# hermeznetwork/circuits

Measured on AMD Instinct MI355X. Metric: rollup-main tx-witnesses/sec (nTx=2048, nLevels=32), higher is better.
Workload: dtype u32x9 (254-bit Montgomery Fr, 29-bit limbs, integer)

## Files before the change

### circuits_amd/csrc/gen/poseidon_consts.inc

```

HZ_CONST_ARR uint32_t HZ_POSEIDON_K_T2[273][9] = {
  {0x01594cdfu, 0x0d359126u, 0x0974b8fau, 0x1c003576u, 0x02471552u, 0x01b4ec3eu, 0x0039cae5u, 0x0c4fdabeu, 0x001abb87u},
  {0x16429dadu, 0x10e8bfb1u, 0x0a355acau, 0x00ddcf00u, 0x157bd068u, 0x1f4bd7c1u, 0x10962bb4u, 0x16de36d0u, 0x000dca6eu},
  {0x1413967du, 0x105a9005u, 0x1046a4bcu, 0x1adfd419u, 0x03171c11u, 0x1a93314fu, 0x19defdc3u, 0x122f21d6u, 0x002ccaaau},
  {0x0c61afc0u, 0x056779b4u, 0x0dee0ab2u, 0x0375598cu, 0x1d6d65a3u, 0x1613901du, 0x0470c410u, 0x1b17f0fau, 0x0012ce74u},
  {0x17380b70u, 0x18b79fd8u, 0x0fff2f50u, 0x1ebcbaa5u, 0x1321aa93u, 0x0b639280u, 0x1f974844u, 0x1c31c015u, 0x00108ac7u},
  {0x1e193ea3u, 0x0edfdd9cu, 0x0997b975u, 0x0df6c0b5u, 0x0217b61fu, 0x19525ecfu, 0x1ab696fau, 0x1fc7b146u, 0x00284e43u},
  {0x1f60828fu, 0x05af232eu, 0x1e6e6a24u, 0x17b52dcau, 0x18396513u, 0x18a70df4u, 0x1ed87095u, 0x1edad4b1u, 0x002aea83u},
  {0x02cda9fbu, 0x1bf0915eu, 0x142bbe4du, 0x13dec3f2u, 0x15bd005fu, 0x1e47caf5u, 0x09d42d28u, 0x1c1453e2u, 0x00070815u},
  {0x0147b227u, 0x043db0d1u, 0x109123eeu, 0x02a96560u, 0x0545d476u, 0x16cafed6u, 0x06a7cde1u, 0x1b289bc1u, 0x000e717bu},
  {0x1245b46cu, 0x05baf901u, 0x158ae172u, 0x02c66a39u, 0x00422146u, 0x0330f8c1u, 0x18ebd100u, 0x083ed501u, 0x00045cd6u},
  {0x1fedd587u, 0x1762b199u, 0x188f8a60u, 0x1a6d7755u, 0x15ecf9b6u, 0x157d5954u, 0x0635d4eau, 0x15bef90du, 0x000f95b8u},
  {0x05977713u, 0x0322e34cu, 0x1952f2aau, 0x160cbb13u, 0x07d0a3afu, 0x0832dff0u, 0x032268dfu, 0x1dd156a4u, 0x00173356u},
  {0x1245b46cu, 0x05baf901u, 0x158ae172u, 0x02c66a39u, 0x00422146u, 0x0330f8c1u, 0x18ebd100u, 0x083ed501u, 0x00045cd6u},
  {0x0a443be3u, 0x0da43148u, 0x0d5bf075u, 0x0aec1b78u, 0x1aaeb7a0u, 0x1ecc745cu, 0x04cf1420u, 0x0dc2926au, 0x002568ccu},
  {0x091b4afcu, 0x1a830c13u, 0x07e0ffd2u, 0x13f0c21au, 0x032af443u, 0x059069deu, 0x00ee1d30u, 0x0b25f8dbu, 0x0023d9c4u},
  {0x199694a7u, 0x12ec6b8au, 0x1aa8f867u, 0x19c45019u, 0x16073cf7u, 0x14374c37u, 0x12acf9a0u, 0x14cc62ffu, 0x001c5cb3u},
  {0x18770d43u, 0x182a6057u, 0x1092ef6bu, 0x1b2c6b34u, 0x0d976099u, 0x09d7d0d6u, 0x10d8175cu, 0x0c978fadu, 0x001490ebu},
  {0x0193c086u, 0x1b408393u, 0x1f3f022au, 0x1a31c81bu, 0x189d54f9u, 0x068b8aa3u, 0x155b774fu, 0x1039e765u, 0x000ba3a7u},
  {0x1245b46cu, 0x05baf901u, 0x158ae172u, 0x02c66a39u, 0x00422146u, 0x0330f8c1u, 0x18ebd100u, 0x083ed501u, 0x00045cd6u},
  {0x1af15785u, 0x11f831e1u, 0x0267daa0u, 0x10300e25u, 0x03e3c029u, 0x0ba31833u, 0x1a77ab80u, 0x10a61ff1u, 0x002819c0u},
  {0x1c17b04du, 0x1e94304eu, 0x068d4e10u, 0x020b4caau, 0x1eae52eeu, 0x1709787au, 0x1d5718cdu, 0x06da8c2cu, 0x000510dfu},
  {0x1245b46cu, 0x05baf901u, 0x158ae172u, 0x02c66a39u, 0x00422146u, 0x0330f8c1u, 0x18ebd100u, 0x083ed501u, 0x00045cd6u},
  {0x034dc162u, 0x1240944bu, 0x11d0aab7u, 0x086e29ddu, 0x0bb57ea5u, 0x1be7bdc5u, 0x1830536bu, 0x0c707f25u, 0x001bae17u},
// ... 444 lines not shown
  {0x0ce9ef2fu, 0x1cccefd1u, 0x107971f9u, 0x18e2974du, 0x08e0fe13u, 0x11069f65u, 0x151cff07u, 0x0529a73cu, 0x0010af75u},
  {0x1c1a175fu, 0x0f3c9877u, 0x0e21d476u, 0x02ac34d1u, 0x0dfef3d2u, 0x064230f2u, 0x08129fddu, 0x18bd622fu, 0x000735e2u},
  {0x0dc8d1cbu, 0x036b8f33u, 0x01ed6b8cu, 0x1eb3968cu, 0x13a7f955u, 0x0864079au, 0x11167e93u, 0x13cb42b8u, 0x0020bc87u},
  {0x13c5e91bu, 0x0ba87ac2u, 0x1b35dd64u, 0x07cee755u, 0x1c0db2ccu, 0x10376d2cu, 0x1fc67e58u, 0x094ac052u, 0x000577e2u},
  {0x06bbddfcu, 0x14337540u, 0x1dc094e9u, 0x124bb7f4u, 0x0e6021a2u, 0x071160b8u, 0x18095154u, 0x02c8ef7fu, 0x002ed3cfu},
  {0x03f43b85u, 0x157841e5u, 0x10c98963u, 0x0418998bu, 0x1937d25eu, 0x0932adcdu, 0x0b54eefbu, 0x131462c1u, 0x0009c178u},
  {0x0ce9ef2fu, 0x1cccefd1u, 0x107971f9u, 0x18e2974du, 0x08e0fe13u, 0x11069f65u, 0x151cff07u, 0x0529a73cu, 0x0010af75u},
  {0x15ee3677u, 0x0c13b231u, 0x144efa88u, 0x0de5b1bfu, 0x1efac993u, 0x151746a9u, 0x14fd0730u, 0x1c09daa0u, 0x001f7c89u},
  {0x1690d1feu, 0x0d1ddecau, 0x1246e6f2u, 0x0b286eedu, 0x1928779cu, 0x1730207cu, 0x03d27a06u, 0x09fc86f6u, 0x003044e2u},
  {0x0ce9ef2fu, 0x1cccefd1u, 0x107971f9u, 0x18e2974du, 0x08e0fe13u, 0x11069f65u, 0x151cff07u, 0x0529a73cu, 0x0010af75u},
  {0x0087dbb8u, 0x0b7f49a5u, 0x17213affu, 0x0169024cu, 0x1efaa808u, 0x1332e2b1u, 0x1c0209aau, 0x03b65ef1u, 0x0029ec7du},
  {0x0dc8d1cbu, 0x036b8f33u, 0x01ed6b8cu, 0x1eb3968cu, 0x13a7f955u, 0x0864079au, 0x11167e93u, 0x13cb42b8u, 0x0020bc87u},
  {0x146627c7u, 0x0ec2014bu, 0x13e3a4fau, 0x10f1fbddu, 0x0c6927bfu, 0x0603e549u, 0x0fdede6bu, 0x04a0114du, 0x002aa135u},
  {0x11130434u, 0x1b3593dfu, 0x19c2e3f3u, 0x191de17eu, 0x174e43cbu, 0x1d73e4a2u, 0x1c6a1356u, 0x090ff16cu, 0x000f7aa8u},
  {0x08c96b43u, 0x15d0d426u, 0x0e9c36cau, 0x101a01f3u, 0x03d48d13u, 0x1b65ca68u, 0x06f3651eu, 0x0e606749u, 0x00014c14u},
  {0x0ce9ef2fu, 0x1cccefd1u, 0x107971f9u, 0x18e2974du, 0x08e0fe13u, 0x11069f65u, 0x151cff07u, 0x0529a73cu, 0x0010af75u},
  {0x1590348du, 0x0b1a1ff0u, 0x0256b576u, 0x0801f689u, 0x175d0092u, 0x06665c08u, 0x1485782bu, 0x0e73a331u, 0x002fe3ecu},
  {0x1b83c1f2u, 0x19d4c354u, 0x09225cd3u, 0x0ff73684u, 0x1a4c9a94u, 0x10d56a72u, 0x048ba310u, 0x1ab2e381u, 0x002c28e9u},
  {0x0ce9ef2fu, 0x1cccefd1u, 0x107971f9u, 0x18e2974du, 0x08e0fe13u, 0x11069f65u, 0x151cff07u, 0x0529a73cu, 0x0010af75u},
  {0x00133bfau, 0x0e899482u, 0x0eafa64du, 0x1ec347e5u, 0x0b3022a6u, 0x0f4f5da0u, 0x03e4545cu, 0x03909282u, 0x002f21f3u},
  {0x0dc8d1cbu, 0x036b8f33u, 0x01ed6b8cu, 0x1eb3968cu, 0x13a7f955u, 0x0864079au, 0x11167e93u, 0x13cb42b8u, 0x0020bc87u},
  {0x0779bf45u, 0x0dd361a6u, 0x114d0302u, 0x1d99ba2eu, 0x186d96c5u, 0x0e36dc9bu, 0x0dcf48feu, 0x1764b264u, 0x000fe0d8u},
  {0x155dba0eu, 0x171c731du, 0x0254bd0au, 0x0e38ebf8u, 0x1826d936u, 0x1a2e087au, 0x028f2facu, 0x1818d078u, 0x00283d8fu},
  {0x01846aafu, 0x03b9a57bu, 0x0f853ed1u, 0x156290a3u, 0x1557be9du, 0x1eeaf251u, 0x0f091d44u, 0x1aab9607u, 0x00089540u},
  {0x0ce9ef2fu, 0x1cccefd1u, 0x107971f9u, 0x18e2974du, 0x08e0fe13u, 0x11069f65u, 0x151cff07u, 0x0529a73cu, 0x0010af75u},
  {0x0aa1dbc3u, 0x14246c75u, 0x1e92c5feu, 0x19c7bb79u, 0x17e27b1du, 0x03f63d37u, 0x0a5d7805u, 0x029841f0u, 0x00082508u},
  {0x03149936u, 0x1f4f4b58u, 0x036104acu, 0x0d90df77u, 0x1716bfedu, 0x1fc8ce86u, 0x02f08225u, 0x074de8acu, 0x00268975u},
  {0x0ce9ef2fu, 0x1cccefd1u, 0x107971f9u, 0x18e2974du, 0x08e0fe13u, 0x11069f65u, 0x151cff07u, 0x0529a73cu, 0x0010af75u},
  {0x0f5596bdu, 0x07513a04u, 0x0be93490u, 0x105ceda5u, 0x09fe80edu, 0x0877ae07u, 0x0ec7a8c6u, 0x1c232985u, 0x002b00bfu},
  {0x0dc8d1cbu, 0x036b8f33u, 0x01ed6b8cu, 0x1eb3968cu, 0x13a7f955u, 0x0864079au, 0x11167e93u, 0x13cb42b8u, 0x0020bc87u},
  {0x16437a6fu, 0x12c5b47bu, 0x1c93eaabu, 0x0bbd1e23u, 0x0ee22d48u, 0x1a99f7ebu, 0x15913e64u, 0x1dbb478bu, 0x00138eadu},
  {0x1f7e1439u, 0x149868dcu, 0x1f3b7c70u, 0x085dd519u, 0x0df0faeau, 0x0c708ff4u, 0x1b3b42a3u, 0x0bb6177fu, 0x00203dcau},
  {0x020ef880u, 0x00aafe94u, 0x01b7bdeau, 0x044c0255u, 0x10f47161u, 0x0450224eu, 0x0a400180u, 0x0b851294u, 0x0018b435u},
  {0x0ce9ef2fu, 0x1cccefd1u, 0x107971f9u, 0x18e2974du, 0x08e0fe13u, 0x11069f65u, 0x151cff07u, 0x0529a73cu, 0x0010af75u},
  {0x0de9c761u, 0x06a21215u, 0x1860e3d0u, 0x1f62786au, 0x1e3ea970u, 0x1ebef040u, 0x0aa65466u, 0x0c3b5683u, 0x0003ee23u},
  {0x145fe787u, 0x00a69c58u, 0x06ffd046u, 0x0586dc35u, 0x0a74d8feu, 0x03266d07u, 0x1af54ed5u, 0x06086d0du, 0x0020c1aeu},
  {0x0ce9ef2fu, 0x1cccefd1u, 0x107971f9u, 0x18e2974du, 0x08e0fe13u, 0x11069f65u, 0x151cff07u, 0x0529a73cu, 0x0010af75u},
  {0x090f1c1au, 0x1dd1e152u, 0x081b956cu, 0x04e3453bu, 0x1ea8f4f6u, 0x02418e5eu, 0x07e022d7u, 0x13bf2ad6u, 0x002275dfu},
  {0x0dc8d1cbu, 0x036b8f33u, 0x01ed6b8cu, 0x1eb3968cu, 0x13a7f955u, 0x0864079au, 0x11167e93u, 0x13cb42b8u, 0x0020bc87u},
  {0x0c1abb13u, 0x1728bdfdu, 0x15074f4au, 0x1a70c65bu, 0x0372a452u, 0x13b51389u, 0x0c3abc69u, 0x0d4a70f3u, 0x0020073au},
  {0x0c2b5d5du, 0x0941df31u, 0x1f9c33bbu, 0x12962a4au, 0x0b917d15u, 0x185a5840u, 0x115784bfu, 0x09080cb2u, 0x000ed415u},
  {0x1775dec2u, 0x15289770u, 0x1c6088a0u, 0x0328b2cdu, 0x11c9218cu, 0x09ef8fc2u, 0x155805e3u, 0x130dcaf3u, 0x000f5a16u},
  {0x0ce9ef2fu, 0x1cccefd1u, 0x107971f9u, 0x18e2974du, 0x08e0fe13u, 0x11069f65u, 0x151cff07u, 0x0529a73cu, 0x0010af75u},
  {0x0f294db4u, 0x060e52fdu, 0x120959ebu, 0x157fdcaeu, 0x0155a8feu, 0x0ca01c37u, 0x03d8b2b0u, 0x0f6f8eeeu, 0x000bb5c3u},
  {0x19a3d3d4u, 0x05c86045u, 0x03d80b84u, 0x1363785cu, 0x0f8cace7u, 0x19750e68u, 0x1c95a3a0u, 0x0b0e3662u, 0x00176155u},
  {0x0ce9ef2fu, 0x1cccefd1u, 0x107971f9u, 0x18e2974du, 0x08e0fe13u, 0x11069f65u, 0x151cff07u, 0x0529a73cu, 0x0010af75u},
  {0x1cdf1c80u, 0x00af0c60u, 0x08f7f367u, 0x05d60c7fu, 0x17e5893cu, 0x0b71ee70u, 0x06987078u, 0x0a699221u, 0x000c359eu},
  {0x0dc8d1cbu, 0x036b8f33u, 0x01ed6b8cu, 0x1eb3968cu, 0x13a7f955u, 0x0864079au, 0x11167e93u, 0x13cb42b8u, 0x0020bc87u},
  {0x187f3b33u, 0x07888857u, 0x02795407u, 0x1f1a4efdu, 0x19cc12ceu, 0x1717fdbdu, 0x1ba7cd83u, 0x0be67905u, 0x00183a79u},
  {0x0a36210du, 0x0bb8a001u, 0x0309ec54u, 0x1a447634u, 0x0f7b6bd7u, 0x04421841u, 0x08805700u, 0x1d4e450bu, 0x00222d33u},
  {0x09ae6794u, 0x03440e85u, 0x03a40f4eu, 0x17aa9436u, 0x0e496c44u, 0x0f93daa8u, 0x0cc6d964u, 0x057a7f72u, 0x00260f79u},
  {0x0ce9ef2fu, 0x1cccefd1u, 0x107971f9u, 0x18e2974du, 0x08e0fe13u, 0x11069f65u, 0x151cff07u, 0x0529a73cu, 0x0010af75u},
  {0x0fe6dd74u, 0x188d3386u, 0x128b4934u, 0x011e4e6fu, 0x178eef24u, 0x01803342u, 0x12b47976u, 0x0ca4122bu, 0x001c86d1u},
  {0x029ab811u, 0x07e39ec6u, 0x1377f398u, 0x07111883u, 0x1565a2b6u, 0x05a895dcu, 0x0c719d0bu, 0x0b6ec86cu, 0x00299cd0u},
  {0x0ce9ef2fu, 0x1cccefd1u, 0x107971f9u, 0x18e2974du, 0x08e0fe13u, 0x11069f65u, 0x151cff07u, 0x0529a73cu, 0x0010af75u},
  {0x13b2c28au, 0x1d65d05au, 0x0669f2a2u, 0x1c2cf4c7u, 0x0558d099u, 0x006d7b4bu, 0x0fd78bb9u, 0x1c3432ceu, 0x002e725cu},
  {0x0dc8d1cbu, 0x036b8f33u, 0x01ed6b8cu, 0x1eb3968cu, 0x13a7f955u, 0x0864079au, 0x11167e93u, 0x13cb42b8u, 0x0020bc87u},
  {0x002ace2bu, 0x082d7fd9u, 0x100eb90bu, 0x05fd2ab3u, 0x0a2ab5a7u, 0x0c503845u, 0x104b1988u, 0x0d86a39eu, 0x00134db8u},
  {0x07e6e8d9u, 0x1f13b995u, 0x1cae0afcu, 0x098a0d09u, 0x12962c84u, 0x0aa5d7a0u, 0x0378ce02u, 0x177cbab4u, 0x000bf75au},
  {0x1e90d55fu, 0x0c21c683u, 0x0a8fdb6eu, 0x026d43d3u, 0x0e390d06u, 0x0d6c90e7u, 0x168d4726u, 0x095549d8u, 0x002a185du},
  {0x0ce9ef2fu, 0x1cccefd1u, 0x107971f9u, 0x18e2974du, 0x08e0fe13u, 0x11069f65u, 0x151cff07u, 0x0529a73cu, 0x0010af75u},
  {0x1fbddbf4u, 0x1304aa18u, 0x088f5eedu, 0x19402e89u, 0x1297e6cdu, 0x1a825ea2u, 0x0f19dcf8u, 0x07a72d6eu, 0x002c1983u},
  {0x07f633bfu, 0x1f9c2a8bu, 0x13a4ce2eu, 0x02ab1954u, 0x0b4efa3au, 0x16ed044fu, 0x0146aa31u, 0x18a3ba03u, 0x0022d34eu},
  {0x0ce9ef2fu, 0x1cccefd1u, 0x107971f9u, 0x18e2974du, 0x08e0fe13u, 0x11069f65u, 0x151cff07u, 0x0529a73cu, 0x0010af75u},
  {0x019b67d0u, 0x164636dcu, 0x126a234au, 0x16d1b300u, 0x1c910526u, 0x0ce66e11u, 0x1e3651e9u, 0x065d025fu, 0x001c3089u},
  {0x0dc8d1cbu, 0x036b8f33u, 0x01ed6b8cu, 0x1eb3968cu, 0x13a7f955u, 0x0864079au, 0x11167e93u, 0x13cb42b8u, 0x0020bc87u},
  {0x0cad4af9u, 0x0b68dc9au, 0x0521d195u, 0x0ca35a05u, 0x1f992f30u, 0x085c9779u, 0x0d2de48bu, 0x1978f12au, 0x0008c9e0u},
  {0x09800555u, 0x113d463bu, 0x069e7f85u, 0x12a0ff18u, 0x14f170a4u, 0x1d0dcc14u, 0x08d21537u, 0x1443adf8u, 0x00293740u},
  {0x00209e79u, 0x0f3754d1u, 0x0a372977u, 0x0af44dacu, 0x1556b961u, 0x02079085u, 0x1689cb71u, 0x062b1b95u, 0x00282c23u},
  {0x1ebad59bu, 0x0303e4d1u, 0x1f9a501eu, 0x0371d097u, 0x1121228bu, 0x030ff9cbu, 0x1669aeebu, 0x17074050u, 0x00167af6u},
  {0x08dedc9cu, 0x105fdd77u, 0x0e4cdd32u, 0x169a2ae2u, 0x183b48d1u, 0x13008989u, 0x1120efb6u, 0x00964973u, 0x001a5077u},
  {0x0db2b350u, 0x12e399dau, 0x0a131677u, 0x029e66cau, 0x05c4c5dfu, 0x0cf59ec0u, 0x15fa74f4u, 0x0fa03f09u, 0x001d5589u},
  {0x08e6a481u, 0x1c20cbc0u, 0x1c586468u, 0x1773f1dfu, 0x1ea21907u, 0x1d0ad80eu, 0x1c95d935u, 0x154be0d5u, 0x000ba91fu},
  {0x1ac99e79u, 0x0b5f4be9u, 0x1916cf2au, 0x0f819302u, 0x023ab1cau, 0x041f93b2u, 0x09cdbbe5u, 0x1fc8875bu, 0x001cd993u},
  {0x0e58f564u, 0x1eef6bf8u, 0x1944e2b1u, 0x164add07u, 0x1b83d866u, 0x17f8882au, 0x1aee24c8u, 0x0691d0ccu, 0x000b299bu},
  {0x1d695ae1u, 0x1c431d9au, 0x1c1f930eu, 0x033e4eb3u, 0x198cfc7bu, 0x1e26027cu, 0x066653dcu, 0x047b3c5bu, 0x000e649eu},
  {0x1f96ed35u, 0x0f49c18fu, 0x1dbb6db8u, 0x1b10e15au, 0x0449aa7du, 0x1e72fce1u, 0x036b8328u, 0x1eb8c773u, 0x0023f542u},
  {0x0ce9ef2fu, 0x1cccefd1u, 0x107971f9u, 0x18e2974du, 0x08e0fe13u, 0x11069f65u, 0x151cff07u, 0x0529a73cu, 0x0010af75u},
  {0x0d9ab9d7u, 0x0ca84190u, 0x04829da9u, 0x132817e3u, 0x17a45765u, 0x1ea14297u, 0x00eb3e80u, 0x061685f7u, 0x001016feu},
  {0x1a861e2du, 0x0e651276u, 0x0ef852f4u, 0x10c58332u, 0x0c3674f3u, 0x16090e81u, 0x0d596687u, 0x1f438e1cu, 0x0013949cu},
  {0x06f7520fu, 0x09d4f250u, 0x15681fe9u, 0x01fcd044u, 0x105154f2u, 0x1a33cff0u, 0x14edfb9fu, 0x19bb1130u, 0x0008a998u},
};
#define HZ_POSEIDON_RP_T2 56
HZ_CONST_ARR uint32_t HZ_POSEIDON_K_T3[407][9] = {
  {0x06950af2u, 0x08df52acu, 0x1f463fb0u, 0x0afd92f8u, 0x14c68fb5u, 0x085357afu, 0x17f37f7du, 0x1a172af8u, 0x00219b98u},
  {0x14ac6331u, 0x19c5c962u, 0x14d4d232u, 0x1b75b979u, 0x05cb57afu, 0x1631c351u, 0x1539ab4eu, 0x0ae57f69u, 0x00221b93u},
  {0x0a11b110u, 0x0dfeef5cu, 0x0072b018u, 0x1dd64482u, 0x001637a2u, 0x1ccbb6f7u, 0x1bfe61e2u, 0x125c529fu, 0x0001ce06u},
  {0x00249cd2u, 0x182cbeffu, 0x156efbbdu, 0x0eba1325u, 0x06ee80ddu, 0x1457c2ebu, 0x0be3d716u, 0x1eff46fcu, 0x00136e88u},
  {0x1072044du, 0x05806d3bu, 0x069a7439u, 0x1dc94561u, 0x0aefed59u, 0x00905741u, 0x049e47f4u, 0x09217d14u, 0x0009b22fu},
  {0x0422baecu, 0x1338c9abu, 0x10cb4a50u, 0x0f33676cu, 0x10e8f39au, 0x12776997u, 0x0d5d7ea2u, 0x1b2dc6aau, 0x002038dfu},
  {0x17bad917u, 0x06dec5c8u, 0x0e531d76u, 0x0c62440bu, 0x147b04a7u, 0x1355af66u, 0x15363704u, 0x06bbd64au, 0x0029f279u},
  {0x0746570du, 0x01d97fc5u, 0x155c6647u, 0x0d79b529u, 0x1b39ce8cu, 0x14086985u, 0x1a8401efu, 0x05c9ac6du, 0x000199b3u},
  {0x09ebbb6cu, 0x1881a596u, 0x181e6e0fu, 0x1fabcdc3u, 0x088b122eu, 0x114f31d0u, 0x0fb3243eu, 0x09ac2ff3u, 0x0012841au},
  {0x1cfff79eu, 0x03d7755du, 0x0552bbd3u, 0x12213286u, 0x09228c55u, 0x0bef4aebu, 0x13fe8d05u, 0x17692838u, 0x00036614u},
  {0x11317367u, 0x1d4e5366u, 0x09855a5du, 0x0c1df16du, 0x0b0de371u, 0x0d9605ccu, 0x0adb0fa5u, 0x1329da0bu, 0x00227fdeu},
  {0x08acea5fu, 0x0838fb1bu, 0x1a12541au, 0x0a38ec24u, 0x02af6162u, 0x188f221fu, 0x19735f0fu, 0x04e9316eu, 0x000e33f9u},
  {0x071e41a6u, 0x08bbea5fu, 0x065da30bu, 0x0228a38au, 0x076a9fb7u, 0x1a1469bdu, 0x114c885eu, 0x110fd199u, 0x001b4b49u},
  {0x0f9e7ad7u, 0x110388bbu, 0x0b23a8beu, 0x0d3738ecu, 0x067c9996u, 0x106d3f50u, 0x0b10e901u, 0x0ec1ca43u, 0x00185422u},
  {0x1d808d1bu, 0x1da4b2b8u, 0x1a384bf5u, 0x0f4905bau, 0x03e20d93u, 0x0012de4fu, 0x121bce86u, 0x16d26544u, 0x000ade3au},
  {0x132d35feu, 0x16391cd7u, 0x16fa00a5u, 0x0bb956dbu, 0x1caed5d5u, 0x1b6e4830u, 0x0a6f14e8u, 0x07466b6cu, 0x00191d6cu},
  {0x012e70d0u, 0x0da73962u, 0x1ec66759u, 0x09107002u, 0x033f84eeu, 0x1399f16eu, 0x0226a56eu, 0x08d116b4u, 0x000e6296u},
  {0x0f9e7ad7u, 0x110388bbu, 0x0b23a8beu, 0x0d3738ecu, 0x067c9996u, 0x106d3f50u, 0x0b10e901u, 0x0ec1ca43u, 0x00185422u},
  {0x0bb951acu, 0x06443faau, 0x17ed611cu, 0x1884421cu, 0x1afce51fu, 0x0efea9e7u, 0x147f1ed0u, 0x0c2df3cfu, 0x00136fbcu},
  {0x1fe33105u, 0x0c4a3c3cu, 0x1c2cdf0fu, 0x041c6828u, 0x048b6c4au, 0x0719d197u, 0x123ecde6u, 0x05abf637u, 0x002ba99eu},
  {0x1137c2e7u, 0x189c540cu, 0x02a348f5u, 0x178dc616u, 0x16997355u, 0x01b921a7u, 0x0fa7ff5fu, 0x02545751u, 0x0009f1ecu},
  {0x13599399u, 0x141ae82bu, 0x13ee16cbu, 0x1358b994u, 0x1601460au, 0x144e8e2fu, 0x0bfd8788u, 0x17aa03a2u, 0x002ae961u},
  {0x05212230u, 0x1c5e5216u, 0x117426b0u, 0x0de4f9e8u, 0x0851a05au, 0x18c6202bu, 0x09247701u, 0x110886d9u, 0x002cb167u},
  {0x18349cb5u, 0x0e276a55u, 0x0cde03c9u, 0x0a96a06cu, 0x02315530u, 0x02cc974fu, 0x15fc8764u, 0x05814578u, 0x0014a31cu},
  {0x03effa5du, 0x162ae321u, 0x14e1d723u, 0x0c68e230u, 0x16cd0944u, 0x1bbee942u, 0x0c6310ddu, 0x11183e90u, 0x002c6b1au},
  {0x05e1c028u, 0x07e01aecu, 0x066688e6u, 0x025ed81cu, 0x14304feau, 0x058a629du, 0x0d6605aeu, 0x173ec4edu, 0x00105204u},
  {0x0f9e7ad7u, 0x110388bbu, 0x0b23a8beu, 0x0d3738ecu, 0x067c9996u, 0x106d3f50u, 0x0b10e901u, 0x0ec1ca43u, 0x00185422u},
  {0x1181abafu, 0x1777b75eu, 0x028f3017u, 0x1c94d28fu, 0x10777d08u, 0x05a1b685u, 0x0a46f0f9u, 0x1e0f866cu, 0x001dbad8u},
  {0x0b3ea51cu, 0x03c81aebu, 0x067c2073u, 0x08738320u, 0x0d32836du, 0x01e483dbu, 0x11cc9a33u, 0x069d55c4u, 0x000f80f1u},
  {0x0fc51587u, 0x0e287af7u, 0x13e1b330u, 0x111abc40u, 0x129058d3u, 0x06ef59b7u, 0x1ea08cafu, 0x0b61be00u, 0x001ec76au},
  {0x0f9e7ad7u, 0x110388bbu, 0x0b23a8beu, 0x0d3738ecu, 0x067c9996u, 0x106d3f50u, 0x0b10e901u, 0x0ec1ca43u, 0x00185422u},
  {0x0df0fb39u, 0x1aa3a276u, 0x1b2456bcu, 0x0b0b4edeu, 0x1ba9e05au, 0x15f65f18u, 0x15794d20u, 0x0cc2d3ecu, 0x00076bd6u},
  {0x13142375u, 0x14870790u, 0x00255288u, 0x1c96ff90u, 0x1fa42dccu, 0x0052b5aau, 0x0670de46u, 0x0cbb0d43u, 0x00260ef0u},
  {0x1137c2e7u, 0x189c540cu, 0x02a348f5u, 0x178dc616u, 0x16997355u, 0x01b921a7u, 0x0fa7ff5fu, 0x02545751u, 0x0009f1ecu},
  {0x0c3aa2dbu, 0x036876d2u, 0x05cbc67bu, 0x162a139du, 0x028bba81u, 0x1b0b894eu, 0x1d398215u, 0x1843792bu, 0x0025435fu},
  {0x08a19517u, 0x1781c4e2u, 0x17c032b7u, 0x0cf6014cu, 0x125fbbc2u, 0x00be09e1u, 0x0291a374u, 0x1080ee7bu, 0x000d2661u},
  {0x044def6eu, 0x15147e38u, 0x060ea740u, 0x0e96aac6u, 0x00fce055u, 0x1356abd6u, 0x1d59ef48u, 0x04b5c547u, 0x00025392u},
  {0x13c28a85u, 0x1744f037u, 0x199f241bu, 0x195989b8u, 0x07693e3bu, 0x09727d90u, 0x000ec272u, 0x0031339au, 0x0011656eu},
  {0x004f4c98u, 0x12aeff7bu, 0x14a4ee7au, 0x189c6531u, 0x1807b4d1u, 0x1fb90164u, 0x0fe8359eu, 0x05aa0bdeu, 0x00143e04u},
  {0x0f9e7ad7u, 0x110388bbu, 0x0b23a8beu, 0x0d3738ecu, 0x067c9996u, 0x106d3f50u, 0x0b10e901u, 0x0ec1ca43u, 0x00185422u},
  {0x0a741350u, 0x1f77effbu, 0x1cdce38au, 0x0658a913u, 0x03783795u, 0x0937fefau, 0x08eeb4f3u, 0x005c1b6au, 0x001188feu},
  {0x09b423d8u, 0x031ea254u, 0x042feb00u, 0x1da37bd7u, 0x140c6fc8u, 0x14a61766u, 0x1745a732u, 0x11d84ceeu, 0x0028ae3fu},
  {0x10751df5u, 0x19b4cf5cu, 0x0bc089e2u, 0x19248dbau, 0x160c19b3u, 0x14de6553u, 0x12ee493cu, 0x097bb0e2u, 0x001dc890u},
  {0x0f9e7ad7u, 0x110388bbu, 0x0b23a8beu, 0x0d3738ecu, 0x067c9996u, 0x106d3f50u, 0x0b10e901u, 0x0ec1ca43u, 0x00185422u},
  {0x193adc08u, 0x16078c77u, 0x06d56e91u, 0x03c2a1efu, 0x1c365a79u, 0x0fd772eau, 0x0827e9eeu, 0x190172bbu, 0x002fd5b0u},
  {0x124638d1u, 0x19c9ba46u, 0x0d3b1c7cu, 0x137e8f4du, 0x03d39810u, 0x1aea945eu, 0x18beb131u, 0x054c38f6u, 0x002e492cu},
  {0x1137c2e7u, 0x189c540cu, 0x02a348f5u, 0x178dc616u, 0x16997355u, 0x01b921a7u, 0x0fa7ff5fu, 0x02545751u, 0x0009f1ecu},
  {0x0ed76c01u, 0x1f2b360au, 0x09540f46u, 0x16ea79a2u, 0x1eb62a52u, 0x0ee0687au, 0x1c4b333bu, 0x1155e835u, 0x001fa7c7u},
  {0x00372895u, 0x04170c43u, 0x1b4cdaa3u, 0x100289ffu, 0x0ed8eb5bu, 0x04452cc9u, 0x02813767u, 0x10470445u, 0x00272319u},
  {0x1c1e81cfu, 0x0e6f1ad7u, 0x1e80f9d4u, 0x0dc77746u, 0x16c3884bu, 0x04e75b8du, 0x07ae2c07u, 0x194253a0u, 0x0004e551u},
  {0x015e9592u, 0x0b0b67c9u, 0x0a6040d5u, 0x1e2118c3u, 0x142bc4ddu, 0x0b213b29u, 0x0ec11bddu, 0x1c2440c0u, 0x000b5732u},
  {0x00b22627u, 0x126f6426u, 0x1ffdba02u, 0x0f2a6ba7u, 0x09a16dfau, 0x1a4f249bu, 0x10de2db9u, 0x0be04320u, 0x00142a4cu},
  {0x0f9e7ad7u, 0x110388bbu, 0x0b23a8beu, 0x0d3738ecu, 0x067c9996u, 0x106d3f50u, 0x0b10e901u, 0x0ec1ca43u, 0x00185422u},
  {0x07d56552u, 0x14c10409u, 0x1bff85c4u, 0x13994671u, 0x0218ce8cu, 0x1070f8dbu, 0x185823d5u, 0x100e7753u, 0x0000847fu},
  {0x16c11742u, 0x14ee17d2u, 0x18e7742eu, 0x0e7c9b5eu, 0x129b3fd1u, 0x020bb1aeu, 0x05569922u, 0x0f07b878u, 0x0017ad0eu},
  {0x03b9a38eu, 0x187e8f4fu, 0x0d3cc940u, 0x03b09c80u, 0x15f75dd3u, 0x160d0e6au, 0x1de9da2bu, 0x115a1843u, 0x00053acbu},
  {0x0f9e7ad7u, 0x110388bbu, 0x0b23a8beu, 0x0d3738ecu, 0x067c9996u, 0x106d3f50u, 0x0b10e901u, 0x0ec1ca43u, 0x00185422u},
  {0x0a0e5b99u, 0x112c0bdau, 0x136ec440u, 0x011bda31u, 0x1e8293b3u, 0x0ed8fffeu, 0x16228411u, 0x1eb9c0a8u, 0x000408f7u},
  {0x0136b0e6u, 0x1b782ae9u, 0x0d4b2341u, 0x09c51220u, 0x0fb1b417u, 0x0135e40eu, 0x08349207u, 0x04817981u, 0x000424ebu},
  {0x1137c2e7u, 0x189c540cu, 0x02a348f5u, 0x178dc616u, 0x16997355u, 0x01b921a7u, 0x0fa7ff5fu, 0x02545751u, 0x0009f1ecu},
  {0x1c058a5cu, 0x11f0f414u, 0x1881b744u, 0x1ea573eeu, 0x0568c0c0u, 0x1461d0f2u, 0x16c672acu, 0x04bf6096u, 0x00115f9au},
  {0x0b3d2dbbu, 0x1f73b37eu, 0x1bdaa8bbu, 0x1dffb532u, 0x1b62d93cu, 0x05493558u, 0x0f951a50u, 0x0f84ad81u, 0x00081e33u},
  {0x19f6b4ddu, 0x1878eef4u, 0x126a20b0u, 0x16fc2d48u, 0x0a7e56cbu, 0x0e4ef340u, 0x0d473220u, 0x0c9d56eeu, 0x0025a632u},
  {0x1bfe70f2u, 0x02b15e7du, 0x0ce8c95du, 0x0a8521ecu, 0x02f9df40u, 0x1cc38b7eu, 0x1d945fb6u, 0x060c100eu, 0x0018f902u},
  {0x18270344u, 0x0b57920fu, 0x1b9c93fdu, 0x03ac7f4cu, 0x1947743bu, 0x17506abbu, 0x16afd566u, 0x1c7dd946u, 0x001fed53u},
  {0x0f9e7ad7u, 0x110388bbu, 0x0b23a8beu, 0x0d3738ecu, 0x067c9996u, 0x106d3f50u, 0x0b10e901u, 0x0ec1ca43u, 0x00185422u},
  {0x1fe0a28du, 0x00078f50u, 0x1478d6e3u, 0x1c0326afu, 0x0134abc1u, 0x14749a6du, 0x1fccfb03u, 0x074f7280u, 0x001afe92u},
  {0x1ddb71d8u, 0x0d176c28u, 0x1a7b6a60u, 0x0e11e3ecu, 0x194df12bu, 0x05fa7958u, 0x0a9400b7u, 0x0dcf9cc5u, 0x0008b5c6u},
  {0x0285585bu, 0x0f4a048du, 0x04237b8fu, 0x1ea6a0e8u, 0x161e90f3u, 0x1e60de4fu, 0x1c3a0eaau, 0x165f0cbeu, 0x00296fc6u},
  {0x0f9e7ad7u, 0x110388bbu, 0x0b23a8beu, 0x0d3738ecu, 0x067c9996u, 0x106d3f50u, 0x0b10e901u, 0x0ec1ca43u, 0x00185422u},
  {0x148bfc35u, 0x0cf89969u, 0x16538c96u, 0x1908b913u, 0x0c80f272u, 0x05cc9d74u, 0x02d2f02eu, 0x1d2c6174u, 0x00269fddu},
  {0x082101f0u, 0x093d5a3cu, 0x1ac61b3du, 0x0ada0389u, 0x02515da2u, 0x0b400f9bu, 0x0879a4a3u, 0x0bfc5fd0u, 0x0011bb73u},
  {0x1137c2e7u, 0x189c540cu, 0x02a348f5u, 0x178dc616u, 0x16997355u, 0x01b921a7u, 0x0fa7ff5fu, 0x02545751u, 0x0009f1ecu},
  {0x1d3c64bcu, 0x03073507u, 0x02a12d0fu, 0x0003f27cu, 0x1f24e51du, 0x1254b14fu, 0x0bee568fu, 0x16003172u, 0x000c42c1u},
  {0x1bddc0d0u, 0x01fd0077u, 0x1bb32ba3u, 0x0715d62cu, 0x05e80565u, 0x15ab3c30u, 0x133f8882u, 0x01185f69u, 0x0017ea3cu},
  {0x0d003002u, 0x0c6e38c7u, 0x0339d8e1u, 0x063769d3u, 0x0b5b9b6eu, 0x1628a5acu, 0x1bbc7ee2u, 0x172584d5u, 0x0001a051u},
  {0x12d02f2bu, 0x1152fc47u, 0x04cb874du, 0x17491130u, 0x1d2e57f2u, 0x0e523b31u, 0x1b098b80u, 0x047d4272u, 0x00267465u},
  {0x1c195f82u, 0x00ce598du, 0x1d0f727fu, 0x07588154u, 0x141ee2dcu, 0x14894b4du, 0x1c441381u, 0x1dd39709u, 0x001bef96u},
  {0x0f9e7ad7u, 0x110388bbu, 0x0b23a8beu, 0x0d3738ecu, 0x067c9996u, 0x106d3f50u, 0x0b10e901u, 0x0ec1ca43u, 0x00185422u},
  {0x1a1739ceu, 0x0f45c151u, 0x02f6c2a2u, 0x0784afa0u, 0x1e3392e7u, 0x04e8f2bdu, 0x091ec827u, 0x10918acdu, 0x002c0081u},
  {0x19836dbfu, 0x1b96e774u, 0x14a9d05fu, 0x1d13244bu, 0x0a5d02c8u, 0x19a2dc16u, 0x092eea4bu, 0x137c7dcbu, 0x000d4079u},
  {0x040174f4u, 0x1c9bcfa0u, 0x1d68236au, 0x1449d35cu, 0x03856edbu, 0x1b6df7a1u, 0x0a6de30cu, 0x089526beu, 0x00183d2fu},
  {0x0f9e7ad7u, 0x110388bbu, 0x0b23a8beu, 0x0d3738ecu, 0x067c9996u, 0x106d3f50u, 0x0b10e901u, 0x0ec1ca43u, 0x00185422u},
// ... 241 lines not shown
  {0x04504510u, 0x0f45d601u, 0x01ecc1b2u, 0x05390587u, 0x18fe614cu, 0x03b9c159u, 0x0e1699b9u, 0x17312ca8u, 0x002c6582u},
  {0x0f9e7ad7u, 0x110388bbu, 0x0b23a8beu, 0x0d3738ecu, 0x067c9996u, 0x106d3f50u, 0x0b10e901u, 0x0ec1ca43u, 0x00185422u},
  {0x17decd6cu, 0x1b512009u, 0x1e9f9256u, 0x19771112u, 0x01f3a959u, 0x02f1eca2u, 0x16707e6fu, 0x111a7d2au, 0x001c8454u},
  {0x1d64b848u, 0x0387544cu, 0x19aa56fdu, 0x0eb4d623u, 0x11edaae2u, 0x16ad2ff1u, 0x07b2692au, 0x167fe61bu, 0x001c6befu},
  {0x1107f769u, 0x13e86f43u, 0x0e096f08u, 0x1d15b2ebu, 0x0583b869u, 0x13dd21dbu, 0x1304cce1u, 0x0a7853a8u, 0x0022f768u},
  {0x0f9e7ad7u, 0x110388bbu, 0x0b23a8beu, 0x0d3738ecu, 0x067c9996u, 0x106d3f50u, 0x0b10e901u, 0x0ec1ca43u, 0x00185422u},
  {0x0d78d317u, 0x0b44e42du, 0x05b02ac4u, 0x15aba253u, 0x1add0fc7u, 0x10327e73u, 0x1ea22c2au, 0x080e44a1u, 0x001db63au},
  {0x054a0314u, 0x087b0914u, 0x16253cf8u, 0x1c9ad78bu, 0x01ed4c61u, 0x0c3a2206u, 0x05de0913u, 0x035ad09fu, 0x002bd824u},
  {0x1137c2e7u, 0x189c540cu, 0x02a348f5u, 0x178dc616u, 0x16997355u, 0x01b921a7u, 0x0fa7ff5fu, 0x02545751u, 0x0009f1ecu},
  {0x16ce8bdbu, 0x0982e0e6u, 0x0f90c5beu, 0x1003a2d6u, 0x1603772au, 0x17d87051u, 0x0f760d39u, 0x015064dbu, 0x001ea2afu},
  {0x106eee6bu, 0x1b1ba868u, 0x169c9c24u, 0x1ff77aa4u, 0x1f68f059u, 0x088f515du, 0x15db4f59u, 0x020b4215u, 0x001541a8u},
  {0x0b2bb3a0u, 0x11f35cf2u, 0x152ff881u, 0x0106230du, 0x0b6d3097u, 0x12149d4du, 0x1116ab6eu, 0x04e4853fu, 0x00085941u},
  {0x0a327e91u, 0x114ba57cu, 0x17d82f7cu, 0x0ef9b1d0u, 0x0134d8fcu, 0x018601e1u, 0x0fff4bb4u, 0x10d507cbu, 0x000f398eu},
  {0x17d2a5f8u, 0x1be95064u, 0x14c2725fu, 0x1cd1e4d0u, 0x01cbaef2u, 0x16ead87du, 0x03e536f9u, 0x0ae8b949u, 0x000c406au},
  {0x0f9e7ad7u, 0x110388bbu, 0x0b23a8beu, 0x0d3738ecu, 0x067c9996u, 0x106d3f50u, 0x0b10e901u, 0x0ec1ca43u, 0x00185422u},
  {0x0c8c189cu, 0x1cc79ae9u, 0x186f6aecu, 0x105d0b36u, 0x01f9589eu, 0x111a0c4eu, 0x09f087f6u, 0x1f316c99u, 0x001e9076u},
  {0x0c8e3650u, 0x0a732d7cu, 0x10ce5b06u, 0x16b2ab83u, 0x19f98e8fu, 0x0c94e3f7u, 0x05f604ceu, 0x1a8b8e0du, 0x0021178du},
  {0x1401e080u, 0x1beb9ea3u, 0x02266b39u, 0x174e8dbcu, 0x1730b2dfu, 0x00f38faau, 0x042c2d23u, 0x1d877771u, 0x0017c9c6u},
  {0x0f9e7ad7u, 0x110388bbu, 0x0b23a8beu, 0x0d3738ecu, 0x067c9996u, 0x106d3f50u, 0x0b10e901u, 0x0ec1ca43u, 0x00185422u},
  {0x1f884e54u, 0x0b9c236fu, 0x0ffa2cfau, 0x0e54ca2du, 0x010c2515u, 0x19c42314u, 0x09e3bc58u, 0x0be5373au, 0x00112560u},
  {0x0ec7d1f5u, 0x087eae30u, 0x1e043f6du, 0x1be1c3a3u, 0x08da1a2du, 0x09b47136u, 0x0e53ffb3u, 0x0a866559u, 0x0016d8a7u},
  {0x1137c2e7u, 0x189c540cu, 0x02a348f5u, 0x178dc616u, 0x16997355u, 0x01b921a7u, 0x0fa7ff5fu, 0x02545751u, 0x0009f1ecu},
  {0x1da30c2cu, 0x0f5d2c4cu, 0x11a6cde7u, 0x116b4311u, 0x1809871au, 0x137d501cu, 0x1123dc35u, 0x1391dbf6u, 0x002d1005u},
  {0x0db8d418u, 0x1adb76f8u, 0x127c029au, 0x14b7d9bdu, 0x17ad4c8bu, 0x17ca7b0du, 0x1d702f41u, 0x1fa8eba5u, 0x002bf205u},
  {0x071418f5u, 0x03adff73u, 0x17631518u, 0x10e4a5efu, 0x0a7296eeu, 0x17fca3f3u, 0x178a4dfdu, 0x0da5e8cau, 0x00012346u},
  {0x11e77690u, 0x13e71dd7u, 0x01d14895u, 0x1db5672du, 0x11b62312u, 0x1cbca505u, 0x093ab4d0u, 0x18eee72eu, 0x001d24f6u},
  {0x09ee2a2du, 0x0ee1c318u, 0x1128c87au, 0x116c5524u, 0x0d79df55u, 0x01c1c1fau, 0x0057112du, 0x1b2fc7d5u, 0x0008fad4u},
  {0x0f9e7ad7u, 0x110388bbu, 0x0b23a8beu, 0x0d3738ecu, 0x067c9996u, 0x106d3f50u, 0x0b10e901u, 0x0ec1ca43u, 0x00185422u},
  {0x01b412a1u, 0x11517daau, 0x00540991u, 0x0113f263u, 0x0cad8dc0u, 0x1e38c735u, 0x1083c0b1u, 0x0454a866u, 0x002de93du},
  {0x066867cbu, 0x1709d8f6u, 0x1268dab4u, 0x1ebf2c12u, 0x04525e2au, 0x15291888u, 0x0572ee91u, 0x169b6e4au, 0x00037f15u},
  {0x0c52838du, 0x1f7616ddu, 0x1ff2c2b6u, 0x0e5b5312u, 0x04fd5bc5u, 0x140fd5f5u, 0x0931bc69u, 0x07ecf7ffu, 0x0010e5b8u},
  {0x0f9e7ad7u, 0x110388bbu, 0x0b23a8beu, 0x0d3738ecu, 0x067c9996u, 0x106d3f50u, 0x0b10e901u, 0x0ec1ca43u, 0x00185422u},
  {0x104007c0u, 0x1973ae9au, 0x17e72900u, 0x1375271bu, 0x1a446a16u, 0x1c953efbu, 0x07d7a070u, 0x1aa59967u, 0x0017f2e5u},
  {0x10581566u, 0x0f7c6f29u, 0x04914c1fu, 0x097c1a30u, 0x11540718u, 0x1b3acacbu, 0x1972e53du, 0x0ce1cb37u, 0x0030293fu},
  {0x1137c2e7u, 0x189c540cu, 0x02a348f5u, 0x178dc616u, 0x16997355u, 0x01b921a7u, 0x0fa7ff5fu, 0x02545751u, 0x0009f1ecu},
  {0x188e3de4u, 0x1f555a7eu, 0x1dd46cdeu, 0x1c6c3570u, 0x1eed9cf2u, 0x0dc8763au, 0x1004454eu, 0x0de3e924u, 0x002f4e33u},
  {0x0c5f88d3u, 0x03e3096au, 0x0f277f99u, 0x002d9412u, 0x0380edcdu, 0x1cf049eau, 0x07298468u, 0x15b6041eu, 0x0009a103u},
  {0x1ea662b3u, 0x19e9c268u, 0x0b673a2fu, 0x0ee34c9cu, 0x0bda421bu, 0x1da6c94du, 0x027e3ec2u, 0x17cf8091u, 0x0011895cu},
  {0x033c4532u, 0x11a0da34u, 0x0e6adaecu, 0x0cf2a6f9u, 0x0ba128b9u, 0x006f2f72u, 0x08cb767du, 0x0b83f781u, 0x000550ecu},
  {0x08083788u, 0x132bf382u, 0x06ab3f3fu, 0x0f45e3c8u, 0x0dd4e47fu, 0x11eeea60u, 0x0704743eu, 0x0d6b3a26u, 0x0009ea97u},
  {0x0f9e7ad7u, 0x110388bbu, 0x0b23a8beu, 0x0d3738ecu, 0x067c9996u, 0x106d3f50u, 0x0b10e901u, 0x0ec1ca43u, 0x00185422u},
  {0x01a5bfb3u, 0x0d5d2e82u, 0x0585a98fu, 0x1607f9f1u, 0x16813062u, 0x0a23f347u, 0x0813c376u, 0x0802503bu, 0x0008fdc2u},
  {0x00645c3cu, 0x05f5f813u, 0x1665816au, 0x1c33f6afu, 0x0fee29c9u, 0x18321ba5u, 0x1a7f3602u, 0x1226e7aeu, 0x0010c633u},
  {0x077a7aafu, 0x174787c6u, 0x16e776d5u, 0x09061190u, 0x17368f18u, 0x0dde5cbeu, 0x10269ba5u, 0x1cc9a02fu, 0x000286f5u},
  {0x0f9e7ad7u, 0x110388bbu, 0x0b23a8beu, 0x0d3738ecu, 0x067c9996u, 0x106d3f50u, 0x0b10e901u, 0x0ec1ca43u, 0x00185422u},
  {0x05e28124u, 0x1b9981d7u, 0x16ae361cu, 0x04bc466bu, 0x1e9aa74bu, 0x1777bd70u, 0x1eb5a877u, 0x1b915a64u, 0x00263302u},
  {0x04736068u, 0x1e6524e9u, 0x0234ea3eu, 0x094ffe5du, 0x12bb81f9u, 0x1c13536eu, 0x02b9f33au, 0x1c536667u, 0x000f5a14u},
  {0x1137c2e7u, 0x189c540cu, 0x02a348f5u, 0x178dc616u, 0x16997355u, 0x01b921a7u, 0x0fa7ff5fu, 0x02545751u, 0x0009f1ecu},
  {0x0a854573u, 0x1ece4e1bu, 0x1a96a584u, 0x1f741153u, 0x17ecba0du, 0x16b912c0u, 0x1f3f28abu, 0x13878f8bu, 0x001478e0u},
  {0x10aaa709u, 0x128030d5u, 0x09db228cu, 0x19a4911fu, 0x10214415u, 0x1d699a6du, 0x1f89f93fu, 0x1ab05164u, 0x00115707u},
  {0x19612a18u, 0x0624738cu, 0x0304ed35u, 0x1a932dccu, 0x039b436bu, 0x093ed15fu, 0x0f91e976u, 0x10efa55fu, 0x000c1d91u},
  {0x1d4373ffu, 0x0885b851u, 0x13bc85ffu, 0x07a97785u, 0x0e01a209u, 0x0a882789u, 0x14f27303u, 0x1f6a17a0u, 0x001f687eu},
  {0x14f3dba6u, 0x1c57a0f3u, 0x15231329u, 0x0906d34cu, 0x1276e7a4u, 0x0647ccb0u, 0x079deceau, 0x1954f267u, 0x001673a3u},
  {0x0f9e7ad7u, 0x110388bbu, 0x0b23a8beu, 0x0d3738ecu, 0x067c9996u, 0x106d3f50u, 0x0b10e901u, 0x0ec1ca43u, 0x00185422u},
  {0x0d1778f7u, 0x041b88deu, 0x08ed1482u, 0x1ab09f93u, 0x11db568fu, 0x1f90934eu, 0x0bd90f32u, 0x07ae718bu, 0x0014be32u},
  {0x18767531u, 0x123587e3u, 0x16cf2177u, 0x0b7a27d5u, 0x199c91e6u, 0x18344467u, 0x1f23001au, 0x1b67428cu, 0x00165fedu},
  {0x04035ab7u, 0x009c7862u, 0x08f75c89u, 0x0e3fd310u, 0x0ddc22c1u, 0x0a209e57u, 0x07e87572u, 0x1a8c9221u, 0x00119157u},
  {0x128dc94bu, 0x19758516u, 0x0b627578u, 0x05c780e8u, 0x05319927u, 0x00faab0au, 0x1a439ee2u, 0x01f5011au, 0x002601a6u},
  {0x1b2e1d77u, 0x08ae3e44u, 0x1d2038d8u, 0x1e635985u, 0x1ae5d306u, 0x13d871bbu, 0x1fbdc1ddu, 0x0f2f62e6u, 0x000059b0u},
  {0x07e732fcu, 0x084df909u, 0x14efe205u, 0x15aa326du, 0x0a20fff7u, 0x17653bacu, 0x02a6c29bu, 0x0b2c5a75u, 0x001f3bc3u},
  {0x048acd07u, 0x03082733u, 0x1e26560au, 0x034af7a5u, 0x0bb2c60bu, 0x163a0e84u, 0x18607102u, 0x001dae37u, 0x002df20fu},
  {0x1600f2beu, 0x019cbdc4u, 0x05a53411u, 0x1d6cdfecu, 0x1739894fu, 0x12a7d77bu, 0x1c6b1d54u, 0x16a08d44u, 0x000bf852u},
  {0x0f99ded2u, 0x0e06bc02u, 0x06df134eu, 0x1578d322u, 0x149724d4u, 0x18c3bf95u, 0x00eae83au, 0x0c011e07u, 0x001750c4u},
  {0x02a052cau, 0x05a87ab0u, 0x14dcddbcu, 0x106decafu, 0x122e2ce8u, 0x03d4082eu, 0x0ef8f873u, 0x1521e336u, 0x0016a065u},
  {0x0df025bau, 0x0ba73f8eu, 0x0f915324u, 0x065bbda3u, 0x0ca80a7cu, 0x118624f1u, 0x09498173u, 0x01c7a1a4u, 0x000af019u},
  {0x05a499dcu, 0x12206bd0u, 0x0b814efbu, 0x0d66bfceu, 0x0e7dbb5cu, 0x0aa0171du, 0x08e70184u, 0x059ef913u, 0x001323dfu},
  {0x0649905eu, 0x17c95f8fu, 0x05a65489u, 0x13644fe0u, 0x0536260au, 0x0ace1d58u, 0x17055235u, 0x06869bfau, 0x001a7e62u},
  {0x0b45af89u, 0x0224c0c3u, 0x1bfb0ddbu, 0x0f9b48f9u, 0x17da019cu, 0x14f45fd8u, 0x10997d57u, 0x0f86e29eu, 0x0026efadu},
  {0x04565569u, 0x07905e05u, 0x1df8e797u, 0x06d4b35bu, 0x04ad02a2u, 0x0778a22fu, 0x01d1297eu, 0x1d84f2a0u, 0x0027fe28u},
  {0x0d82889au, 0x0fa45e0eu, 0x1bd530f5u, 0x1a53f924u, 0x05eb0d8au, 0x1b365b8bu, 0x1381f308u, 0x196c0c25u, 0x001bede7u},
  {0x0bec1d0cu, 0x04b3688eu, 0x18cf405fu, 0x0f800727u, 0x056de992u, 0x00fb9fd2u, 0x05514427u, 0x1fb2f130u, 0x0020c03fu},
  {0x01768fb6u, 0x18f63897u, 0x070ed03cu, 0x1a001f72u, 0x04ce0399u, 0x01841053u, 0x0b9737e5u, 0x09292366u, 0x0010faecu},
  {0x0751cdcau, 0x0fe2d7e2u, 0x0162e9f3u, 0x0b12636cu, 0x05f02906u, 0x1a592918u, 0x17c0c8beu, 0x003c4496u, 0x001a52bdu},
  {0x0e8efa33u, 0x0f51cc96u, 0x0edc3d40u, 0x12573aefu, 0x16b95ae8u, 0x1b7bf14fu, 0x011482afu, 0x16b1e719u, 0x00135a61u},
  {0x0f9e7ad7u, 0x110388bbu, 0x0b23a8beu, 0x0d3738ecu, 0x067c9996u, 0x106d3f50u, 0x0b10e901u, 0x0ec1ca43u, 0x00185422u},
  {0x1d808d1bu, 0x1da4b2b8u, 0x1a384bf5u, 0x0f4905bau, 0x03e20d93u, 0x0012de4fu, 0x121bce86u, 0x16d26544u, 0x000ade3au},
  {0x132d35feu, 0x16391cd7u, 0x16fa00a5u, 0x0bb956dbu, 0x1caed5d5u, 0x1b6e4830u, 0x0a6f14e8u, 0x07466b6cu, 0x00191d6cu},
  {0x18e9ba8fu, 0x1d8162aeu, 0x0fbf09d7u, 0x168662d1u, 0x0ef7b2feu, 0x015d7d55u, 0x09195718u, 0x0267a28cu, 0x000fe908u},
  {0x04f388d7u, 0x01b14590u, 0x1598e8a8u, 0x12c58329u, 0x115458c8u, 0x13a62935u, 0x03d65e2eu, 0x13e8407cu, 0x000ab495u},
  {0x0564e591u, 0x01d4df72u, 0x0b0ad8d6u, 0x1655ae03u, 0x13a1b5e6u, 0x0a93bc0du, 0x16ec5d74u, 0x1374ea59u, 0x002369d6u},
  {0x0004eaddu, 0x05365bf4u, 0x0493016eu, 0x1d1a2414u, 0x0c60826du, 0x023b2076u, 0x026fd3e9u, 0x055a47d6u, 0x0021dc8bu},
  {0x17fddfa0u, 0x161a5176u, 0x030d78bau, 0x15ef8400u, 0x08d839abu, 0x1b2dce76u, 0x14b8a677u, 0x07c85cffu, 0x000877ecu},
  {0x0e5224f4u, 0x1e27ada2u, 0x1eb9ae97u, 0x0a2f7a59u, 0x1f07c890u, 0x1a2da267u, 0x05d3f5a1u, 0x11654cdeu, 0x000ba411u},
};
HZ_CONST_ARR uint32_t HZ_POSEIDON_KW_T3[407][9] = {
  {0x06950af2u, 0x08df52acu, 0x1f463fb0u, 0x0afd92f8u, 0x14c68fb5u, 0x085357afu, 0x17f37f7du, 0x1a172af8u, 0x00219b98u},
  {0x14ac6331u, 0x19c5c962u, 0x14d4d232u, 0x1b75b979u, 0x05cb57afu, 0x1631c351u, 0x1539ab4eu, 0x0ae57f69u, 0x00221b93u},
  {0x0a11b110u, 0x0dfeef5cu, 0x0072b018u, 0x1dd64482u, 0x001637a2u, 0x1ccbb6f7u, 0x1bfe61e2u, 0x125c529fu, 0x0001ce06u},
  {0x00249cd2u, 0x182cbeffu, 0x156efbbdu, 0x0eba1325u, 0x06ee80ddu, 0x1457c2ebu, 0x0be3d716u, 0x1eff46fcu, 0x00136e88u},
  {0x1072044du, 0x05806d3bu, 0x069a7439u, 0x1dc94561u, 0x0aefed59u, 0x00905741u, 0x049e47f4u, 0x09217d14u, 0x0009b22fu},
  {0x0422baecu, 0x1338c9abu, 0x10cb4a50u, 0x0f33676cu, 0x10e8f39au, 0x12776997u, 0x0d5d7ea2u, 0x1b2dc6aau, 0x002038dfu},
  {0x17bad917u, 0x06dec5c8u, 0x0e531d76u, 0x0c62440bu, 0x147b04a7u, 0x1355af66u, 0x15363704u, 0x06bbd64au, 0x0029f279u},
  {0x0746570du, 0x01d97fc5u, 0x155c6647u, 0x0d79b529u, 0x1b39ce8cu, 0x14086985u, 0x1a8401efu, 0x05c9ac6du, 0x000199b3u},
  {0x09ebbb6cu, 0x1881a596u, 0x181e6e0fu, 0x1fabcdc3u, 0x088b122eu, 0x114f31d0u, 0x0fb3243eu, 0x09ac2ff3u, 0x0012841au},
  {0x1cfff79eu, 0x03d7755du, 0x0552bbd3u, 0x12213286u, 0x09228c55u, 0x0bef4aebu, 0x13fe8d05u, 0x17692838u, 0x00036614u},
  {0x11317367u, 0x1d4e5366u, 0x09855a5du, 0x0c1df16du, 0x0b0de371u, 0x0d9605ccu, 0x0adb0fa5u, 0x1329da0bu, 0x00227fdeu},
  {0x08acea5fu, 0x0838fb1bu, 0x1a12541au, 0x0a38ec24u, 0x02af6162u, 0x188f221fu, 0x19735f0fu, 0x04e9316eu, 0x000e33f9u},
  {0x071e41a6u, 0x08bbea5fu, 0x065da30bu, 0x0228a38au, 0x076a9fb7u, 0x1a1469bdu, 0x114c885eu, 0x110fd199u, 0x001b4b49u},
  {0x1a4711d7u, 0x16699559u, 0x1c235d50u, 0x0b4e4a8eu, 0x14df94adu, 0x0965c795u, 0x1d7afd37u, 0x0342cc8du, 0x002d76dbu},
  {0x1d808d1bu, 0x1da4b2b8u, 0x1a384bf5u, 0x0f4905bau, 0x03e20d93u, 0x0012de4fu, 0x121bce86u, 0x16d26544u, 0x000ade3au},
  {0x132d35feu, 0x16391cd7u, 0x16fa00a5u, 0x0bb956dbu, 0x1caed5d5u, 0x1b6e4830u, 0x0a6f14e8u, 0x07466b6cu, 0x00191d6cu},
  {0x012e70d0u, 0x0da73962u, 0x1ec66759u, 0x09107002u, 0x033f84eeu, 0x1399f16eu, 0x0226a56eu, 0x08d116b4u, 0x000e6296u},
  {0x1a4711d7u, 0x16699559u, 0x1c235d50u, 0x0b4e4a8eu, 0x14df94adu, 0x0965c795u, 0x1d7afd37u, 0x0342cc8du, 0x002d76dbu},
  {0x0bb951acu, 0x06443faau, 0x17ed611cu, 0x1884421cu, 0x1afce51fu, 0x0efea9e7u, 0x147f1ed0u, 0x0c2df3cfu, 0x00136fbcu},
  {0x1fe33105u, 0x0c4a3c3cu, 0x1c2cdf0fu, 0x041c6828u, 0x048b6c4au, 0x0719d197u, 0x123ecde6u, 0x05abf637u, 0x002ba99eu},
  {0x068a4cfdu, 0x1fd63110u, 0x13da84bdu, 0x0a050f73u, 0x028bc9fcu, 0x1f7d6d37u, 0x06270e37u, 0x18ff0e31u, 0x001cf5b4u},
  {0x13599399u, 0x141ae82bu, 0x13ee16cbu, 0x1358b994u, 0x1601460au, 0x144e8e2fu, 0x0bfd8788u, 0x17aa03a2u, 0x002ae961u},
  {0x14725df5u, 0x1b005648u, 0x0162c706u, 0x0531cd6du, 0x02a601f6u, 0x165a1032u, 0x162de27fu, 0x05fe8aa5u, 0x002ddc1bu},
  {0x1726ad0au, 0x1fd8b292u, 0x09a1fb0fu, 0x151b5e74u, 0x0fe81d33u, 0x06afb3b4u, 0x0d979567u, 0x02e791a9u, 0x000c050bu},
  {0x196992a9u, 0x1d5a94c8u, 0x1c410c4cu, 0x1872c758u, 0x06ccf87au, 0x050d05b8u, 0x0620aa0eu, 0x1febdc6au, 0x000503fdu},
  {0x14832d19u, 0x0c864124u, 0x142a6f13u, 0x1d21efa1u, 0x12b9569eu, 0x066ca828u, 0x044dcb54u, 0x02a472afu, 0x002ee064u},
  {0x1a4711d7u, 0x16699559u, 0x1c235d50u, 0x0b4e4a8eu, 0x14df94adu, 0x0965c795u, 0x1d7afd37u, 0x0342cc8du, 0x002d76dbu},
  {0x1181abafu, 0x1777b75eu, 0x028f3017u, 0x1c94d28fu, 0x10777d08u, 0x05a1b685u, 0x0a46f0f9u, 0x1e0f866cu, 0x001dbad8u},
  {0x0b3ea51cu, 0x03c81aebu, 0x067c2073u, 0x08738320u, 0x0d32836du, 0x01e483dbu, 0x11cc9a33u, 0x069d55c4u, 0x000f80f1u},
  {0x0fc51587u, 0x0e287af7u, 0x13e1b330u, 0x111abc40u, 0x129058d3u, 0x06ef59b7u, 0x1ea08cafu, 0x0b61be00u, 0x001ec76au},
  {0x1a4711d7u, 0x16699559u, 0x1c235d50u, 0x0b4e4a8eu, 0x14df94adu, 0x0965c795u, 0x1d7afd37u, 0x0342cc8du, 0x002d76dbu},
  {0x0df0fb39u, 0x1aa3a276u, 0x1b2456bcu, 0x0b0b4edeu, 0x1ba9e05au, 0x15f65f18u, 0x15794d20u, 0x0cc2d3ecu, 0x00076bd6u},
  {0x13142375u, 0x14870790u, 0x00255288u, 0x1c96ff90u, 0x1fa42dccu, 0x0052b5aau, 0x0670de46u, 0x0cbb0d43u, 0x00260ef0u},
  {0x068a4cfdu, 0x1fd63110u, 0x13da84bdu, 0x0a050f73u, 0x028bc9fcu, 0x1f7d6d37u, 0x06270e37u, 0x18ff0e31u, 0x001cf5b4u},
  {0x0c3aa2dbu, 0x036876d2u, 0x05cbc67bu, 0x162a139du, 0x028bba81u, 0x1b0b894eu, 0x1d398215u, 0x1843792bu, 0x0025435fu},
  {0x137a33b7u, 0x03f5fbbbu, 0x121af88eu, 0x1d01a9f8u, 0x0d6390b5u, 0x026b6983u, 0x0413bb1bu, 0x1856e380u, 0x000d084fu},
  {0x1d0d9ecbu, 0x097a305fu, 0x01130901u, 0x10506c2bu, 0x0896c878u, 0x16684f5au, 0x1aa3ac6bu, 0x119611f1u, 0x00118237u},
  {0x12d676c8u, 0x06ed38b8u, 0x017fa970u, 0x0ed10765u, 0x1f0efb44u, 0x0a05ba6cu, 0x03e3151bu, 0x14e1bd7au, 0x001dc77bu},
  {0x18219b9bu, 0x1954cd82u, 0x13d500cau, 0x182aa853u, 0x0a6d8b14u, 0x0cde9933u, 0x17244744u, 0x19c86591u, 0x002459b7u},
  {0x1a4711d7u, 0x16699559u, 0x1c235d50u, 0x0b4e4a8eu, 0x14df94adu, 0x0965c795u, 0x1d7afd37u, 0x0342cc8du, 0x002d76dbu},
  {0x0a741350u, 0x1f77effbu, 0x1cdce38au, 0x0658a913u, 0x03783795u, 0x0937fefau, 0x08eeb4f3u, 0x005c1b6au, 0x001188feu},
  {0x09b423d8u, 0x031ea254u, 0x042feb00u, 0x1da37bd7u, 0x140c6fc8u, 0x14a61766u, 0x1745a732u, 0x11d84ceeu, 0x0028ae3fu},
  {0x10751df5u, 0x19b4cf5cu, 0x0bc089e2u, 0x19248dbau, 0x160c19b3u, 0x14de6553u, 0x12ee493cu, 0x097bb0e2u, 0x001dc890u},
  {0x1a4711d7u, 0x16699559u, 0x1c235d50u, 0x0b4e4a8eu, 0x14df94adu, 0x0965c795u, 0x1d7afd37u, 0x0342cc8du, 0x002d76dbu},
  {0x193adc08u, 0x16078c77u, 0x06d56e91u, 0x03c2a1efu, 0x1c365a79u, 0x0fd772eau, 0x0827e9eeu, 0x190172bbu, 0x002fd5b0u},
  {0x124638d1u, 0x19c9ba46u, 0x0d3b1c7cu, 0x137e8f4du, 0x03d39810u, 0x1aea945eu, 0x18beb131u, 0x054c38f6u, 0x002e492cu},
  {0x068a4cfdu, 0x1fd63110u, 0x13da84bdu, 0x0a050f73u, 0x028bc9fcu, 0x1f7d6d37u, 0x06270e37u, 0x18ff0e31u, 0x001cf5b4u},
  {0x0ed76c01u, 0x1f2b360au, 0x09540f46u, 0x16ea79a2u, 0x1eb62a52u, 0x0ee0687au, 0x1c4b333bu, 0x1155e835u, 0x001fa7c7u},
  {0x0c84cfb7u, 0x0f60856fu, 0x01250caau, 0x03df44b0u, 0x0a88cc23u, 0x089a9e40u, 0x199df927u, 0x197e3d72u, 0x00090b50u},
  {0x07ed5296u, 0x08309766u, 0x13d285ddu, 0x101efe56u, 0x18535a20u, 0x04b4e7a8u, 0x18e7fa88u, 0x15feb658u, 0x0021dae6u},
  {0x0f4ab17fu, 0x1133e7ceu, 0x0eb88ffbu, 0x15087e81u, 0x1a7eadadu, 0x1d0a26b1u, 0x1957d717u, 0x0d7bcd9fu, 0x001f589eu},
  {0x06462a0du, 0x02b7344bu, 0x0ad5c140u, 0x1af91cb0u, 0x0ddd502fu, 0x0a37b18cu, 0x045c4737u, 0x1c40f96eu, 0x0011c7c8u},
  {0x1a4711d7u, 0x16699559u, 0x1c235d50u, 0x0b4e4a8eu, 0x14df94adu, 0x0965c795u, 0x1d7afd37u, 0x0342cc8du, 0x002d76dbu},
  {0x07d56552u, 0x14c10409u, 0x1bff85c4u, 0x13994671u, 0x0218ce8cu, 0x1070f8dbu, 0x185823d5u, 0x100e7753u, 0x0000847fu},
  {0x16c11742u, 0x14ee17d2u, 0x18e7742eu, 0x0e7c9b5eu, 0x129b3fd1u, 0x020bb1aeu, 0x05569922u, 0x0f07b878u, 0x0017ad0eu},
  {0x03b9a38eu, 0x187e8f4fu, 0x0d3cc940u, 0x03b09c80u, 0x15f75dd3u, 0x160d0e6au, 0x1de9da2bu, 0x115a1843u, 0x00053acbu},
  {0x1a4711d7u, 0x16699559u, 0x1c235d50u, 0x0b4e4a8eu, 0x14df94adu, 0x0965c795u, 0x1d7afd37u, 0x0342cc8du, 0x002d76dbu},
  {0x0a0e5b99u, 0x112c0bdau, 0x136ec440u, 0x011bda31u, 0x1e8293b3u, 0x0ed8fffeu, 0x16228411u, 0x1eb9c0a8u, 0x000408f7u},
  {0x0136b0e6u, 0x1b782ae9u, 0x0d4b2341u, 0x09c51220u, 0x0fb1b417u, 0x0135e40eu, 0x08349207u, 0x04817981u, 0x000424ebu},
  {0x068a4cfdu, 0x1fd63110u, 0x13da84bdu, 0x0a050f73u, 0x028bc9fcu, 0x1f7d6d37u, 0x06270e37u, 0x18ff0e31u, 0x001cf5b4u},
  {0x1c058a5cu, 0x11f0f414u, 0x1881b744u, 0x1ea573eeu, 0x0568c0c0u, 0x1461d0f2u, 0x16c672acu, 0x04bf6096u, 0x00115f9au},
  {0x094ebfd4u, 0x0d47c9a8u, 0x15ea20f3u, 0x08317642u, 0x170adfcau, 0x1fcd5fcbu, 0x04c99096u, 0x111c32aau, 0x002e5c83u},
  {0x1802183eu, 0x07e52223u, 0x1446cd28u, 0x15e69cbfu, 0x02ced7a1u, 0x0de9a90eu, 0x0535631eu, 0x0f20adffu, 0x000d259bu},
  {0x1d308172u, 0x0ad59071u, 0x085cb467u, 0x1e36a0bdu, 0x04198146u, 0x1a21c1c8u, 0x0b64b510u, 0x0b0adc5du, 0x0025dd52u},
  {0x1e2da772u, 0x00835255u, 0x0955e640u, 0x09c71077u, 0x1a87db02u, 0x04d66f25u, 0x1ec156d8u, 0x12625712u, 0x001dcc16u},
  {0x1a4711d7u, 0x16699559u, 0x1c235d50u, 0x0b4e4a8eu, 0x14df94adu, 0x0965c795u, 0x1d7afd37u, 0x0342cc8du, 0x002d76dbu},
  {0x1fe0a28du, 0x00078f50u, 0x1478d6e3u, 0x1c0326afu, 0x0134abc1u, 0x14749a6du, 0x1fccfb03u, 0x074f7280u, 0x001afe92u},
  {0x1ddb71d8u, 0x0d176c28u, 0x1a7b6a60u, 0x0e11e3ecu, 0x194df12bu, 0x05fa7958u, 0x0a9400b7u, 0x0dcf9cc5u, 0x0008b5c6u},
  {0x0285585bu, 0x0f4a048du, 0x04237b8fu, 0x1ea6a0e8u, 0x161e90f3u, 0x1e60de4fu, 0x1c3a0eaau, 0x165f0cbeu, 0x00296fc6u},
  {0x1a4711d7u, 0x16699559u, 0x1c235d50u, 0x0b4e4a8eu, 0x14df94adu, 0x0965c795u, 0x1d7afd37u, 0x0342cc8du, 0x002d76dbu},
  {0x148bfc35u, 0x0cf89969u, 0x16538c96u, 0x1908b913u, 0x0c80f272u, 0x05cc9d74u, 0x02d2f02eu, 0x1d2c6174u, 0x00269fddu},
  {0x082101f0u, 0x093d5a3cu, 0x1ac61b3du, 0x0ada0389u, 0x02515da2u, 0x0b400f9bu, 0x0879a4a3u, 0x0bfc5fd0u, 0x0011bb73u},
  {0x068a4cfdu, 0x1fd63110u, 0x13da84bdu, 0x0a050f73u, 0x028bc9fcu, 0x1f7d6d37u, 0x06270e37u, 0x18ff0e31u, 0x001cf5b4u},
  {0x1d3c64bcu, 0x03073507u, 0x02a12d0fu, 0x0003f27cu, 0x1f24e51du, 0x1254b14fu, 0x0bee568fu, 0x16003172u, 0x000c42c1u},
  {0x0e28a5dfu, 0x14aaf111u, 0x01500700u, 0x17ae740bu, 0x1823e1abu, 0x0941469eu, 0x1cd9e9a3u, 0x089fcaa3u, 0x001a9340u},
  {0x1fe953dbu, 0x1b0550b2u, 0x113081e2u, 0x1ce1ad77u, 0x1cc23c0bu, 0x19862292u, 0x07da7441u, 0x14604074u, 0x00122b00u},
  {0x189360ccu, 0x00f4d6cfu, 0x05c64a62u, 0x041f5b88u, 0x09e749a9u, 0x06b022ddu, 0x0fba7039u, 0x083eca6cu, 0x002ad2b4u},
  {0x104fc2a8u, 0x1119d1c0u, 0x148ffc7eu, 0x127830eeu, 0x043bc94cu, 0x189532b9u, 0x0183862eu, 0x04ac30c8u, 0x000bf3fdu},
  {0x1a4711d7u, 0x16699559u, 0x1c235d50u, 0x0b4e4a8eu, 0x14df94adu, 0x0965c795u, 0x1d7afd37u, 0x0342cc8du, 0x002d76dbu},
  {0x1a1739ceu, 0x0f45c151u, 0x02f6c2a2u, 0x0784afa0u, 0x1e3392e7u, 0x04e8f2bdu, 0x091ec827u, 0x10918acdu, 0x002c0081u},
  {0x19836dbfu, 0x1b96e774u, 0x14a9d05fu, 0x1d13244bu, 0x0a5d02c8u, 0x19a2dc16u, 0x092eea4bu, 0x137c7dcbu, 0x000d4079u},
  {0x040174f4u, 0x1c9bcfa0u, 0x1d68236au, 0x1449d35cu, 0x03856edbu, 0x1b6df7a1u, 0x0a6de30cu, 0x089526beu, 0x00183d2fu},
  {0x1a4711d7u, 0x16699559u, 0x1c235d50u, 0x0b4e4a8eu, 0x14df94adu, 0x0965c795u, 0x1d7afd37u, 0x0342cc8du, 0x002d76dbu},
// ... 241 lines not shown
  {0x185c06e6u, 0x1acd2060u, 0x09f13546u, 0x1632c012u, 0x0adb560bu, 0x1f8f83fdu, 0x043970c4u, 0x090568b9u, 0x002bafe9u},
  {0x1a4711d7u, 0x16699559u, 0x1c235d50u, 0x0b4e4a8eu, 0x14df94adu, 0x0965c795u, 0x1d7afd37u, 0x0342cc8du, 0x002d76dbu},
  {0x17decd6cu, 0x1b512009u, 0x1e9f9256u, 0x19771112u, 0x01f3a959u, 0x02f1eca2u, 0x16707e6fu, 0x111a7d2au, 0x001c8454u},
  {0x1d64b848u, 0x0387544cu, 0x19aa56fdu, 0x0eb4d623u, 0x11edaae2u, 0x16ad2ff1u, 0x07b2692au, 0x167fe61bu, 0x001c6befu},
  {0x1107f769u, 0x13e86f43u, 0x0e096f08u, 0x1d15b2ebu, 0x0583b869u, 0x13dd21dbu, 0x1304cce1u, 0x0a7853a8u, 0x0022f768u},
  {0x1a4711d7u, 0x16699559u, 0x1c235d50u, 0x0b4e4a8eu, 0x14df94adu, 0x0965c795u, 0x1d7afd37u, 0x0342cc8du, 0x002d76dbu},
  {0x0d78d317u, 0x0b44e42du, 0x05b02ac4u, 0x15aba253u, 0x1add0fc7u, 0x10327e73u, 0x1ea22c2au, 0x080e44a1u, 0x001db63au},
  {0x054a0314u, 0x087b0914u, 0x16253cf8u, 0x1c9ad78bu, 0x01ed4c61u, 0x0c3a2206u, 0x05de0913u, 0x035ad09fu, 0x002bd824u},
  {0x068a4cfdu, 0x1fd63110u, 0x13da84bdu, 0x0a050f73u, 0x028bc9fcu, 0x1f7d6d37u, 0x06270e37u, 0x18ff0e31u, 0x001cf5b4u},
  {0x16ce8bdbu, 0x0982e0e6u, 0x0f90c5beu, 0x1003a2d6u, 0x1603772au, 0x17d87051u, 0x0f760d39u, 0x015064dbu, 0x001ea2afu},
  {0x1a011c44u, 0x0749d3adu, 0x19e7538fu, 0x127ace8bu, 0x075228a1u, 0x167999beu, 0x1d281b9bu, 0x009c7303u, 0x00109532u},
  {0x1a5cb872u, 0x1611fcf1u, 0x18eba770u, 0x135f5e04u, 0x07248222u, 0x04b684fcu, 0x188fc050u, 0x12d1f064u, 0x0018b335u},
  {0x0dfc7eeeu, 0x000279f5u, 0x1df140deu, 0x05fdd766u, 0x1dae1aeau, 0x0854346eu, 0x0c97665cu, 0x19c5a768u, 0x000eeb44u},
  {0x08694e5eu, 0x1da9de00u, 0x09edcd95u, 0x19d3b050u, 0x18b26442u, 0x09453651u, 0x1e4d9868u, 0x1853c5dfu, 0x001e2384u},
  {0x1a4711d7u, 0x16699559u, 0x1c235d50u, 0x0b4e4a8eu, 0x14df94adu, 0x0965c795u, 0x1d7afd37u, 0x0342cc8du, 0x002d76dbu},
  {0x0c8c189cu, 0x1cc79ae9u, 0x186f6aecu, 0x105d0b36u, 0x01f9589eu, 0x111a0c4eu, 0x09f087f6u, 0x1f316c99u, 0x001e9076u},
  {0x0c8e3650u, 0x0a732d7cu, 0x10ce5b06u, 0x16b2ab83u, 0x19f98e8fu, 0x0c94e3f7u, 0x05f604ceu, 0x1a8b8e0du, 0x0021178du},
  {0x1401e080u, 0x1beb9ea3u, 0x02266b39u, 0x174e8dbcu, 0x1730b2dfu, 0x00f38faau, 0x042c2d23u, 0x1d877771u, 0x0017c9c6u},
  {0x1a4711d7u, 0x16699559u, 0x1c235d50u, 0x0b4e4a8eu, 0x14df94adu, 0x0965c795u, 0x1d7afd37u, 0x0342cc8du, 0x002d76dbu},
  {0x1f884e54u, 0x0b9c236fu, 0x0ffa2cfau, 0x0e54ca2du, 0x010c2515u, 0x19c42314u, 0x09e3bc58u, 0x0be5373au, 0x00112560u},
  {0x0ec7d1f5u, 0x087eae30u, 0x1e043f6du, 0x1be1c3a3u, 0x08da1a2du, 0x09b47136u, 0x0e53ffb3u, 0x0a866559u, 0x0016d8a7u},
  {0x068a4cfdu, 0x1fd63110u, 0x13da84bdu, 0x0a050f73u, 0x028bc9fcu, 0x1f7d6d37u, 0x06270e37u, 0x18ff0e31u, 0x001cf5b4u},
  {0x1da30c2cu, 0x0f5d2c4cu, 0x11a6cde7u, 0x116b4311u, 0x1809871au, 0x137d501cu, 0x1123dc35u, 0x1391dbf6u, 0x002d1005u},
  {0x1bd0e9e8u, 0x16c855dbu, 0x122e30e2u, 0x0a45d15eu, 0x164b0017u, 0x00c91fb5u, 0x0b383caeu, 0x0192821du, 0x0027a242u},
  {0x061088e5u, 0x06ad42d3u, 0x1c3f9509u, 0x1e26bbd2u, 0x1d4b96f4u, 0x0029432cu, 0x0ac30fe0u, 0x106015e7u, 0x00012ff4u},
  {0x13387124u, 0x07da2b39u, 0x11632bccu, 0x1fa87b21u, 0x16cbe30au, 0x1c3a66e8u, 0x056b0585u, 0x1d20ee10u, 0x0013c2cau},
  {0x1c110a8du, 0x105aa29eu, 0x06b50424u, 0x01576549u, 0x046d2ba7u, 0x03f1043cu, 0x0e483368u, 0x0a83e681u, 0x001ccdbbu},
  {0x1a4711d7u, 0x16699559u, 0x1c235d50u, 0x0b4e4a8eu, 0x14df94adu, 0x0965c795u, 0x1d7afd37u, 0x0342cc8du, 0x002d76dbu},
  {0x01b412a1u, 0x11517daau, 0x00540991u, 0x0113f263u, 0x0cad8dc0u, 0x1e38c735u, 0x1083c0b1u, 0x0454a866u, 0x002de93du},
  {0x066867cbu, 0x1709d8f6u, 0x1268dab4u, 0x1ebf2c12u, 0x04525e2au, 0x15291888u, 0x0572ee91u, 0x169b6e4au, 0x00037f15u},
  {0x0c52838du, 0x1f7616ddu, 0x1ff2c2b6u, 0x0e5b5312u, 0x04fd5bc5u, 0x140fd5f5u, 0x0931bc69u, 0x07ecf7ffu, 0x0010e5b8u},
  {0x1a4711d7u, 0x16699559u, 0x1c235d50u, 0x0b4e4a8eu, 0x14df94adu, 0x0965c795u, 0x1d7afd37u, 0x0342cc8du, 0x002d76dbu},
  {0x104007c0u, 0x1973ae9au, 0x17e72900u, 0x1375271bu, 0x1a446a16u, 0x1c953efbu, 0x07d7a070u, 0x1aa59967u, 0x0017f2e5u},
  {0x10581566u, 0x0f7c6f29u, 0x04914c1fu, 0x097c1a30u, 0x11540718u, 0x1b3acacbu, 0x1972e53du, 0x0ce1cb37u, 0x0030293fu},
  {0x068a4cfdu, 0x1fd63110u, 0x13da84bdu, 0x0a050f73u, 0x028bc9fcu, 0x1f7d6d37u, 0x06270e37u, 0x18ff0e31u, 0x001cf5b4u},
  {0x188e3de4u, 0x1f555a7eu, 0x1dd46cdeu, 0x1c6c3570u, 0x1eed9cf2u, 0x0dc8763au, 0x1004454eu, 0x0de3e924u, 0x002f4e33u},
  {0x0428e26eu, 0x1dfcca49u, 0x0a255f58u, 0x1d4729dcu, 0x11ad1818u, 0x16ac8f76u, 0x1a617988u, 0x07c3cbd7u, 0x00137e6cu},
  {0x1a677934u, 0x1b4972cau, 0x172cc7b7u, 0x1c0e2766u, 0x05efa07eu, 0x05646c56u, 0x03df9d04u, 0x0e76e86au, 0x002f0c44u},
  {0x0c6a0b5au, 0x147c7d1au, 0x0bbe7543u, 0x036aaf5du, 0x0be9f4a3u, 0x1df62ebbu, 0x1f9b1f9du, 0x1aba29e7u, 0x0020748cu},
  {0x1a5871dcu, 0x1107d65du, 0x108a1034u, 0x06cb6d1du, 0x1d6b979eu, 0x1636d657u, 0x17942459u, 0x0abd8bc1u, 0x0020d7a3u},
  {0x1a4711d7u, 0x16699559u, 0x1c235d50u, 0x0b4e4a8eu, 0x14df94adu, 0x0965c795u, 0x1d7afd37u, 0x0342cc8du, 0x002d76dbu},
  {0x01a5bfb3u, 0x0d5d2e82u, 0x0585a98fu, 0x1607f9f1u, 0x16813062u, 0x0a23f347u, 0x0813c376u, 0x0802503bu, 0x0008fdc2u},
  {0x00645c3cu, 0x05f5f813u, 0x1665816au, 0x1c33f6afu, 0x0fee29c9u, 0x18321ba5u, 0x1a7f3602u, 0x1226e7aeu, 0x0010c633u},
  {0x077a7aafu, 0x174787c6u, 0x16e776d5u, 0x09061190u, 0x17368f18u, 0x0dde5cbeu, 0x10269ba5u, 0x1cc9a02fu, 0x000286f5u},
  {0x1a4711d7u, 0x16699559u, 0x1c235d50u, 0x0b4e4a8eu, 0x14df94adu, 0x0965c795u, 0x1d7afd37u, 0x0342cc8du, 0x002d76dbu},
  {0x05e28124u, 0x1b9981d7u, 0x16ae361cu, 0x04bc466bu, 0x1e9aa74bu, 0x1777bd70u, 0x1eb5a877u, 0x1b915a64u, 0x00263302u},
  {0x04736068u, 0x1e6524e9u, 0x0234ea3eu, 0x094ffe5du, 0x12bb81f9u, 0x1c13536eu, 0x02b9f33au, 0x1c536667u, 0x000f5a14u},
  {0x068a4cfdu, 0x1fd63110u, 0x13da84bdu, 0x0a050f73u, 0x028bc9fcu, 0x1f7d6d37u, 0x06270e37u, 0x18ff0e31u, 0x001cf5b4u},
  {0x0a854573u, 0x1ece4e1bu, 0x1a96a584u, 0x1f741153u, 0x17ecba0du, 0x16b912c0u, 0x1f3f28abu, 0x13878f8bu, 0x001478e0u},
  {0x10e5f1f3u, 0x157794d0u, 0x0df662bbu, 0x0e9ea2fbu, 0x1d54b5aau, 0x1d54c61fu, 0x1c2b025cu, 0x0753e560u, 0x000ea082u},
  {0x0e50a7c1u, 0x038d14e7u, 0x11e65ea8u, 0x18cddbc4u, 0x0c14c302u, 0x10781784u, 0x08c24800u, 0x00d12802u, 0x00079c82u},
  {0x12ac3722u, 0x0808bddeu, 0x1aaae71fu, 0x1a7a3d48u, 0x129d6642u, 0x085fd886u, 0x03792c26u, 0x165ed284u, 0x0011a5adu},
  {0x0f3d9038u, 0x1d27260eu, 0x180a8f6eu, 0x13d27264u, 0x07876c4eu, 0x010dd03fu, 0x15e7f8d5u, 0x0a86bb97u, 0x002adf72u},
  {0x1a4711d7u, 0x16699559u, 0x1c235d50u, 0x0b4e4a8eu, 0x14df94adu, 0x0965c795u, 0x1d7afd37u, 0x0342cc8du, 0x002d76dbu},
  {0x0d1778f7u, 0x041b88deu, 0x08ed1482u, 0x1ab09f93u, 0x11db568fu, 0x1f90934eu, 0x0bd90f32u, 0x07ae718bu, 0x0014be32u},
  {0x18767531u, 0x123587e3u, 0x16cf2177u, 0x0b7a27d5u, 0x199c91e6u, 0x18344467u, 0x1f23001au, 0x1b67428cu, 0x00165fedu},
  {0x0b194c0fu, 0x1c36032fu, 0x058a911fu, 0x1de2d1e9u, 0x098ecd60u, 0x147e6eadu, 0x013bf6a7u, 0x11bf8046u, 0x00141e04u},
  {0x049390ddu, 0x00c1ee47u, 0x13c46350u, 0x14549337u, 0x07dddfd7u, 0x1c0300b3u, 0x0dc28459u, 0x009dc7efu, 0x000d87ebu},
  {0x1b2e1d77u, 0x08ae3e44u, 0x1d2038d8u, 0x1e635985u, 0x1ae5d306u, 0x13d871bbu, 0x1fbdc1ddu, 0x0f2f62e6u, 0x000059b0u},
  {0x07e732fcu, 0x084df909u, 0x14efe205u, 0x15aa326du, 0x0a20fff7u, 0x17653bacu, 0x02a6c29bu, 0x0b2c5a75u, 0x001f3bc3u},
  {0x048acd07u, 0x03082733u, 0x1e26560au, 0x034af7a5u, 0x0bb2c60bu, 0x163a0e84u, 0x18607102u, 0x001dae37u, 0x002df20fu},
  {0x1600f2beu, 0x019cbdc4u, 0x05a53411u, 0x1d6cdfecu, 0x1739894fu, 0x12a7d77bu, 0x1c6b1d54u, 0x16a08d44u, 0x000bf852u},
  {0x0f99ded2u, 0x0e06bc02u, 0x06df134eu, 0x1578d322u, 0x149724d4u, 0x18c3bf95u, 0x00eae83au, 0x0c011e07u, 0x001750c4u},
  {0x02a052cau, 0x05a87ab0u, 0x14dcddbcu, 0x106decafu, 0x122e2ce8u, 0x03d4082eu, 0x0ef8f873u, 0x1521e336u, 0x0016a065u},
  {0x0df025bau, 0x0ba73f8eu, 0x0f915324u, 0x065bbda3u, 0x0ca80a7cu, 0x118624f1u, 0x09498173u, 0x01c7a1a4u, 0x000af019u},
  {0x05a499dcu, 0x12206bd0u, 0x0b814efbu, 0x0d66bfceu, 0x0e7dbb5cu, 0x0aa0171du, 0x08e70184u, 0x059ef913u, 0x001323dfu},
  {0x0649905eu, 0x17c95f8fu, 0x05a65489u, 0x13644fe0u, 0x0536260au, 0x0ace1d58u, 0x17055235u, 0x06869bfau, 0x001a7e62u},
  {0x0b45af89u, 0x0224c0c3u, 0x1bfb0ddbu, 0x0f9b48f9u, 0x17da019cu, 0x14f45fd8u, 0x10997d57u, 0x0f86e29eu, 0x0026efadu},
  {0x04565569u, 0x07905e05u, 0x1df8e797u, 0x06d4b35bu, 0x04ad02a2u, 0x0778a22fu, 0x01d1297eu, 0x1d84f2a0u, 0x0027fe28u},
  {0x0d82889au, 0x0fa45e0eu, 0x1bd530f5u, 0x1a53f924u, 0x05eb0d8au, 0x1b365b8bu, 0x1381f308u, 0x196c0c25u, 0x001bede7u},
  {0x0bec1d0cu, 0x04b3688eu, 0x18cf405fu, 0x0f800727u, 0x056de992u, 0x00fb9fd2u, 0x05514427u, 0x1fb2f130u, 0x0020c03fu},
  {0x01768fb6u, 0x18f63897u, 0x070ed03cu, 0x1a001f72u, 0x04ce0399u, 0x01841053u, 0x0b9737e5u, 0x09292366u, 0x0010faecu},
  {0x0751cdcau, 0x0fe2d7e2u, 0x0162e9f3u, 0x0b12636cu, 0x05f02906u, 0x1a592918u, 0x17c0c8beu, 0x003c4496u, 0x001a52bdu},
  {0x0e8efa33u, 0x0f51cc96u, 0x0edc3d40u, 0x12573aefu, 0x16b95ae8u, 0x1b7bf14fu, 0x011482afu, 0x16b1e719u, 0x00135a61u},
  {0x1a4711d7u, 0x16699559u, 0x1c235d50u, 0x0b4e4a8eu, 0x14df94adu, 0x0965c795u, 0x1d7afd37u, 0x0342cc8du, 0x002d76dbu},
  {0x1e8e62ebu, 0x03a16563u, 0x076a3d7cu, 0x0073c17eu, 0x18f52010u, 0x0c82c216u, 0x1cbe05fcu, 0x025958adu, 0x00041786u},
  {0x05f5c4c3u, 0x046c833cu, 0x0da83f13u, 0x11600f96u, 0x1bde836cu, 0x12f8c600u, 0x0e24e04cu, 0x043055c1u, 0x0012876fu},
  {0x07a2c19bu, 0x05a11638u, 0x064680abu, 0x0b142b1du, 0x198b0c85u, 0x0d0c9cb9u, 0x1b92ab93u, 0x1e961003u, 0x00109c78u},
  {0x1ae38379u, 0x10bea467u, 0x054dc1a2u, 0x0756210du, 0x1f4d8becu, 0x1edd5f6au, 0x0a597893u, 0x108b6c43u, 0x002c2b43u},
  {0x13e0bee8u, 0x14a7b653u, 0x1c05c6ecu, 0x071d949fu, 0x0341b2c2u, 0x0a31366eu, 0x01529ee0u, 0x068a7c28u, 0x0008ae3cu},
  {0x06ca4b2bu, 0x0f221bc1u, 0x192f0137u, 0x033b3288u, 0x113c2166u, 0x07e5114du, 0x08d44449u, 0x1771f3efu, 0x000e08d9u},
  {0x0686d883u, 0x004f59bdu, 0x1b05a390u, 0x0d931b7cu, 0x1494c930u, 0x17dcce38u, 0x17d324a5u, 0x09f221bfu, 0x002856b1u},
  {0x009c1bbau, 0x0bdaaccdu, 0x19620decu, 0x1ed4065bu, 0x1d8de23eu, 0x105fb12au, 0x00059d0fu, 0x14ff9303u, 0x0004a081u},
};
#define HZ_POSEIDON_RP_T3 57
HZ_CONST_ARR uint32_t HZ_POSEIDON_K_T4[533][9] = {
  {0x1974a4aau, 0x173f8237u, 0x01c6c311u, 0x085b63b7u, 0x1ebada24u, 0x193abce2u, 0x0170f8f7u, 0x08aaa948u, 0x002e82b5u},
  {0x1d102cf4u, 0x0c47a55bu, 0x1bf54b21u, 0x12d68a24u, 0x0a8fb796u, 0x0802b49eu, 0x0b131270u, 0x0c0053a1u, 0x00138914u},
  {0x03001832u, 0x1b63e925u, 0x1b7bdaa9u, 0x19f02793u, 0x063e0c01u, 0x190b6547u, 0x133868b8u, 0x0ca80b70u, 0x0009e04fu},
  {0x1e6bcab8u, 0x0e88a801u, 0x0424b9e2u, 0x132cd069u, 0x17f3b58du, 0x07539679u, 0x18dae88cu, 0x10beca0du, 0x00114004u},
  {0x0f9b0c5bu, 0x17e62397u, 0x0976d376u, 0x1aa867afu, 0x0700943cu, 0x188c5bdfu, 0x1d6de597u, 0x15a35b32u, 0x002ea3bau},
  {0x0ce0a86au, 0x09e37bb7u, 0x1d68878cu, 0x0b1d84bdu, 0x1fcd67c2u, 0x146f30acu, 0x1c30812eu, 0x1442527bu, 0x000d983eu},
  {0x06764474u, 0x1f69c479u, 0x0af89c43u, 0x04fe2543u, 0x13eda3b7u, 0x1bb8db0cu, 0x1efb46acu, 0x0ebd3d52u, 0x000304acu},
  {0x1e20ee9du, 0x11baed21u, 0x098c120cu, 0x16530153u, 0x158a4e55u, 0x032caca6u, 0x01f3d943u, 0x145d363au, 0x0023635du},
  {0x134e6995u, 0x11bc197du, 0x1b188686u, 0x148e10bcu, 0x1ac8133au, 0x14342782u, 0x133d8a08u, 0x13309d02u, 0x00157132u},
  {0x0c750e13u, 0x036f5806u, 0x1f4bd7a0u, 0x0539cc65u, 0x02cbd3c6u, 0x178e147du, 0x1a9fa892u, 0x08590845u, 0x001be7c5u},
  {0x09f4b49au, 0x16c2c649u, 0x0353ee2fu, 0x1425f454u, 0x1aa52bf9u, 0x0c42d883u, 0x1c8a191au, 0x109169edu, 0x002ac240u},
  {0x0ad7947cu, 0x03580443u, 0x04ad42aeu, 0x0a72455bu, 0x03af5194u, 0x13fec652u, 0x0706059fu, 0x01eeb6d7u, 0x000fc831u},
  {0x0a562518u, 0x0d791fa0u, 0x19490b37u, 0x158c9733u, 0x1b568d0eu, 0x07e9d4f3u, 0x1ef2520du, 0x0c90c4b4u, 0x000bae49u},
  {0x07d03f76u, 0x001fcd4eu, 0x04e169cfu, 0x00b6a478u, 0x1d04e8dbu, 0x0f1151c1u, 0x1f6bc2f7u, 0x077a6448u, 0x001e57f8u},
  {0x061b9a73u, 0x0510047fu, 0x1572a721u, 0x1bd1dd06u, 0x0ee70ac9u, 0x1ed24fadu, 0x026b8b30u, 0x09c8166fu, 0x00285e9fu},
  {0x1fffcd36u, 0x16f193edu, 0x0142e1d4u, 0x0c2d28fbu, 0x10e05d86u, 0x1be829b1u, 0x003a976fu, 0x0da6bfbfu, 0x002f7c4du},
  {0x0c6335e1u, 0x105b024fu, 0x1f701d16u, 0x121ec6dcu, 0x1a44c83au, 0x02146f9bu, 0x136407cfu, 0x1f0ed39eu, 0x00119c12u},
  {0x03983252u, 0x13f83131u, 0x1f9fc1ccu, 0x113045adu, 0x17d34ee6u, 0x08144bc5u, 0x158d4f6du, 0x075ac18du, 0x00227e77u},
  {0x17b7fb4au, 0x167c5b86u, 0x0899d116u, 0x1245a399u, 0x16c5abbfu, 0x171f805bu, 0x0e8ec159u, 0x1ad34859u, 0x00014bccu},
  {0x189162c0u, 0x0d922f6du, 0x07fc12c1u, 0x12d07117u, 0x04a47191u, 0x09ce4429u, 0x0abefc92u, 0x18624fc8u, 0x000f573bu},
  {0x0254986eu, 0x1011ec2du, 0x05ce9f36u, 0x1787335fu, 0x160994bcu, 0x04d68de3u, 0x157b5ec8u, 0x18b1d95fu, 0x0007ec5du},
  {0x05893698u, 0x1842ef62u, 0x0389920cu, 0x16f05f15u, 0x15cdb6bbu, 0x0848342du, 0x0a2a1c43u, 0x1b84c55eu, 0x0025a328u},
  {0x03983252u, 0x13f83131u, 0x1f9fc1ccu, 0x113045adu, 0x17d34ee6u, 0x08144bc5u, 0x158d4f6du, 0x075ac18du, 0x00227e77u},
  {0x14fcea58u, 0x1b981a42u, 0x03fd24ceu, 0x1068aa46u, 0x1c2d010au, 0x0c36b928u, 0x11fdd2bfu, 0x111150e1u, 0x000bcf1du},
  {0x0c7e04b2u, 0x1cd634edu, 0x156bc341u, 0x0f328577u, 0x1e17d456u, 0x1be5e816u, 0x04e3ab42u, 0x0c00fe57u, 0x0017d827u},
  {0x1cc951e1u, 0x02b1db35u, 0x08ce7a41u, 0x034f197bu, 0x11d6a66eu, 0x1cf79159u, 0x1034570du, 0x045df826u, 0x000d4a8du},
  {0x028975e1u, 0x08440b73u, 0x1bf5d7afu, 0x0fa08600u, 0x178348bau, 0x00a54d11u, 0x0bd05bb8u, 0x01510da2u, 0x002a4591u},
  {0x0e43527au, 0x1a261341u, 0x06c2e9fcu, 0x1a2cfc73u, 0x0ec67b6bu, 0x12a1ab65u, 0x07fb666cu, 0x177c5771u, 0x0007a34fu},
  {0x1aeb686du, 0x17692d8eu, 0x13ea59e4u, 0x095e7538u, 0x1f75ed58u, 0x19484bccu, 0x0d48fbecu, 0x1a98d47fu, 0x000a3234u},
  {0x146c11f1u, 0x0a50c67du, 0x128cfd25u, 0x1f094544u, 0x1a3c8ef3u, 0x10cb0d69u, 0x145d2b30u, 0x1a6fdbd6u, 0x002dcb60u},
  {0x05ee93d0u, 0x06a5b39bu, 0x0782a455u, 0x0664578eu, 0x14930f9du, 0x0a6ef0d8u, 0x050d65d6u, 0x111d7d2cu, 0x00094d9cu},
  {0x0dbb37b4u, 0x1914e204u, 0x1dd7a210u, 0x1db500ccu, 0x1d3876b1u, 0x1d912e97u, 0x16062115u, 0x0c7d26adu, 0x002425a4u},
  {0x17226295u, 0x0d96ac07u, 0x08a9f07bu, 0x011c2ee0u, 0x03380eaeu, 0x02e8eca4u, 0x061d1893u, 0x0c65b706u, 0x0013fb71u},
  {0x0faa86a2u, 0x14070cd9u, 0x174d5144u, 0x13794a5cu, 0x105a78d6u, 0x11be4e4du, 0x0e6bfaa2u, 0x1b7c624au, 0x0002ab62u},
  {0x03983252u, 0x13f83131u, 0x1f9fc1ccu, 0x113045adu, 0x17d34ee6u, 0x08144bc5u, 0x158d4f6du, 0x075ac18du, 0x00227e77u},
  {0x1498cc2eu, 0x14bf59f2u, 0x17dce654u, 0x01598cc1u, 0x06ed42afu, 0x055eb673u, 0x0727ada6u, 0x02e38d18u, 0x001b7a88u},
  {0x087efd3eu, 0x165873e1u, 0x0a14c92bu, 0x00f4cf67u, 0x02c16a37u, 0x0e8b18d5u, 0x1f7bb655u, 0x131e3e30u, 0x0012ccceu},
  {0x12ce0922u, 0x060f893bu, 0x0ae07c66u, 0x177dfd2eu, 0x17185561u, 0x12bbb853u, 0x1020a488u, 0x136432b9u, 0x00248e40u},
  {0x1a935a20u, 0x0b22ebb3u, 0x04300d64u, 0x057fd686u, 0x1b79e13au, 0x1fc89e13u, 0x11d2e994u, 0x08b418d0u, 0x001b3dcau},
  {0x03983252u, 0x13f83131u, 0x1f9fc1ccu, 0x113045adu, 0x17d34ee6u, 0x08144bc5u, 0x158d4f6du, 0x075ac18du, 0x00227e77u},
  {0x016bc902u, 0x09885ddbu, 0x0a4f6fddu, 0x120b7bb7u, 0x1165f6d9u, 0x0ce8d688u, 0x1f99dd9eu, 0x0629e168u, 0x002f27a8u},
  {0x1c61c748u, 0x1663cf37u, 0x191056beu, 0x1dce1039u, 0x18941e6eu, 0x022cf43cu, 0x11d26058u, 0x16416ddcu, 0x00003000u},
  {0x0b6ef0d9u, 0x13da2457u, 0x16451902u, 0x113a46ecu, 0x0949dca3u, 0x05d390e4u, 0x1dfc5e8eu, 0x186ab112u, 0x002b210bu},
  {0x028975e1u, 0x08440b73u, 0x1bf5d7afu, 0x0fa08600u, 0x178348bau, 0x00a54d11u, 0x0bd05bb8u, 0x01510da2u, 0x002a4591u},
  {0x016e7355u, 0x0c26c48cu, 0x079059d1u, 0x1a721c44u, 0x0c08fa83u, 0x167616e5u, 0x151397cau, 0x154172a9u, 0x000ff058u},
  {0x196fcdb6u, 0x1a5bd507u, 0x0f02016au, 0x12a7e4c5u, 0x1ac5e8b3u, 0x136ccb0bu, 0x0ec99404u, 0x17a34c61u, 0x002df7f2u},
  {0x166348a0u, 0x18416a6bu, 0x11b5e841u, 0x139935c4u, 0x1020c073u, 0x1d346238u, 0x0a2f832bu, 0x1a770106u, 0x001b8aebu},
  {0x104144cbu, 0x0f6845d6u, 0x1da87543u, 0x1b3153f8u, 0x08ed220fu, 0x1bfe5c92u, 0x0a09acc5u, 0x092c0dbcu, 0x002f5643u},
  {0x178bcc03u, 0x0e3d6756u, 0x1dbb70bfu, 0x1888d513u, 0x0eebd6e8u, 0x061bc41cu, 0x07ae5f8au, 0x0afd893eu, 0x001038f9u},
  {0x115daa94u, 0x118574bdu, 0x1483d3aeu, 0x0225e45du, 0x1609f9e3u, 0x161a3d15u, 0x1dda443cu, 0x132286bbu, 0x002fbcb3u},
  {0x1c9396d8u, 0x038904c6u, 0x09b2bf52u, 0x07c6b380u, 0x10af6e5du, 0x0c5ae65bu, 0x1a8fd9deu, 0x0eec2903u, 0x0003d0b3u},
  {0x03983252u, 0x13f83131u, 0x1f9fc1ccu, 0x113045adu, 0x17d34ee6u, 0x08144bc5u, 0x158d4f6du, 0x075ac18du, 0x00227e77u},
  {0x1160b872u, 0x03be55d9u, 0x0aa5a955u, 0x16bcbebfu, 0x15afdbe2u, 0x1dac1277u, 0x0906d994u, 0x0d6ee700u, 0x00115763u},
  {0x017aed25u, 0x034e126eu, 0x0a0625feu, 0x1ea27c9cu, 0x09a0b080u, 0x1f5b534fu, 0x1e57c3b9u, 0x10d0151eu, 0x001c5231u},
  {0x143f878eu, 0x00cc275fu, 0x00c16773u, 0x1d49a431u, 0x0ce72f85u, 0x0ecd88ebu, 0x109a9a6du, 0x04ee45e3u, 0x0011cabfu},
  {0x0ff30f41u, 0x00e20e11u, 0x08c95d84u, 0x0b792c4au, 0x0a3955d1u, 0x0d0a2592u, 0x1cfd7b51u, 0x07b16e15u, 0x0011f889u},
  {0x03983252u, 0x13f83131u, 0x1f9fc1ccu, 0x113045adu, 0x17d34ee6u, 0x08144bc5u, 0x158d4f6du, 0x075ac18du, 0x00227e77u},
  {0x1df36f99u, 0x0ab16535u, 0x1166c443u, 0x0fa2c174u, 0x0f70f712u, 0x1101348cu, 0x1e972bfeu, 0x0add472cu, 0x001c9f05u},
  {0x09556a32u, 0x0703a295u, 0x037b2fcbu, 0x0932afcfu, 0x145732dfu, 0x1a5e3118u, 0x0a95dd40u, 0x17e9b178u, 0x002551b5u},
  {0x189c07b0u, 0x0c856e96u, 0x0ad8fb9cu, 0x02841aa5u, 0x19320f5cu, 0x0dcd21c5u, 0x120365fbu, 0x07d7173au, 0x000e2bb5u},
  {0x028975e1u, 0x08440b73u, 0x1bf5d7afu, 0x0fa08600u, 0x178348bau, 0x00a54d11u, 0x0bd05bb8u, 0x01510da2u, 0x002a4591u},
  {0x0293f0a5u, 0x06693c4fu, 0x00ea5c35u, 0x103fbcc6u, 0x09aec2c6u, 0x0c9ab580u, 0x15f6baaau, 0x09241f2fu, 0x001744f0u},
  {0x19ba6abau, 0x04fbfd71u, 0x120b105bu, 0x0846f7f5u, 0x13cb8571u, 0x05f2c2a1u, 0x1b571bdeu, 0x07332637u, 0x000d2b67u},
  {0x0aa685e9u, 0x042722e4u, 0x0eb10239u, 0x121c8f42u, 0x160afcfcu, 0x1137d01bu, 0x033be137u, 0x0048e7e9u, 0x0001e1d7u},
  {0x0073ea8bu, 0x0581f3c8u, 0x07a8907au, 0x1fe612e8u, 0x1c7fa638u, 0x04b9461eu, 0x1aa1d3fdu, 0x1fb83662u, 0x001c8048u},
  {0x073b74ddu, 0x1e30561bu, 0x13e3273du, 0x11324fc5u, 0x12dc9eafu, 0x0820223au, 0x11c87d5bu, 0x1f2e0495u, 0x00034cffu},
  {0x0d4f2993u, 0x0fb67511u, 0x080d1fa4u, 0x0f8df3e7u, 0x1c252dfdu, 0x129ddf43u, 0x0ef444c7u, 0x0bd7de58u, 0x0027ad88u},
  {0x1b79e4b2u, 0x095d71f0u, 0x0cf4d8b8u, 0x0a95f0d9u, 0x0d763459u, 0x16fc2659u, 0x17898069u, 0x12c9de58u, 0x000a0b82u},
  {0x03983252u, 0x13f83131u, 0x1f9fc1ccu, 0x113045adu, 0x17d34ee6u, 0x08144bc5u, 0x158d4f6du, 0x075ac18du, 0x00227e77u},
  {0x1b31dbebu, 0x18f82bd8u, 0x018391dau, 0x14a08dd6u, 0x1ac8c3ddu, 0x1aa4ef4cu, 0x125ea72fu, 0x0c3dc3d5u, 0x00048b10u},
  {0x1ae7b258u, 0x03f0bff8u, 0x188559d5u, 0x1cddd834u, 0x097a9e02u, 0x111b02a3u, 0x01e9fcc2u, 0x1bcd72bdu, 0x0009e5fau},
  {0x0ef579aau, 0x08eed31fu, 0x0ac46ffcu, 0x19da8290u, 0x0dd01b4bu, 0x08d96ccfu, 0x1fac90d4u, 0x1588e3bau, 0x00133a56u},
  {0x0e1c2991u, 0x181d1d89u, 0x01fc32d1u, 0x06dd3b78u, 0x1e9d1dd0u, 0x09c91960u, 0x057147c5u, 0x1a5120a4u, 0x000117b1u},
  {0x03983252u, 0x13f83131u, 0x1f9fc1ccu, 0x113045adu, 0x17d34ee6u, 0x08144bc5u, 0x158d4f6du, 0x075ac18du, 0x00227e77u},
  {0x1ef54eccu, 0x08c43a00u, 0x096cf550u, 0x080a8e2au, 0x0d492c8cu, 0x1830d986u, 0x169b85beu, 0x07b9f3fdu, 0x002a8fcfu},
  {0x1078268du, 0x09f26959u, 0x06730450u, 0x104c767du, 0x0e485395u, 0x1549c13cu, 0x0ed62be4u, 0x14e3f0cbu, 0x002bcd41u},
  {0x00cef7c7u, 0x1b944816u, 0x091c0340u, 0x15741362u, 0x14bad92du, 0x0b37e7d4u, 0x0e660115u, 0x028d00a6u, 0x001059c5u},
  {0x028975e1u, 0x08440b73u, 0x1bf5d7afu, 0x0fa08600u, 0x178348bau, 0x00a54d11u, 0x0bd05bb8u, 0x01510da2u, 0x002a4591u},
  {0x18e91fdau, 0x0d7e23ecu, 0x10574c1bu, 0x0f0f2f27u, 0x0f2065dau, 0x1019b1eeu, 0x0f1d2a23u, 0x1960443fu, 0x0025f1a2u},
  {0x148d69dau, 0x1f13bbfbu, 0x1052eefcu, 0x1f03ff82u, 0x1e21b955u, 0x165ae53eu, 0x14e0db9cu, 0x1a821604u, 0x00269ce3u},
// ... 6500 lines not shown
```

### circuits_amd/csrc/poseidon.h

```cpp
#pragma once
#include "fr.h"

namespace hz {

template <int T>
struct PoseidonCfg;
template <> struct PoseidonCfg<2> { static constexpr int RP = 56; };
template <> struct PoseidonCfg<3> { static constexpr int RP = 57; };
template <> struct PoseidonCfg<4> { static constexpr int RP = 56; };
template <> struct PoseidonCfg<5> { static constexpr int RP = 60; };
template <> struct PoseidonCfg<6> { static constexpr int RP = 60; };
template <> struct PoseidonCfg<7> { static constexpr int RP = 63; };

template <int T> constexpr int poseidon_rounds() { return 8 + PoseidonCfg<T>::RP; }
template <int T> constexpr int poseidon_nsbox() { return 8 * T + PoseidonCfg<T>::RP; }

template <int T> constexpr int poseidon_k_e0() { return 4 * T; }
template <int T> constexpr int poseidon_k_part() { return 4 * T + 1; }
template <int T> constexpr int poseidon_k_dense() {
    return poseidon_k_part<T>() + (PoseidonCfg<T>::RP / 2) * (4 * T + 1) + (PoseidonCfg<T>::RP % 2) * 2 * T;
}
template <int T> constexpr int poseidon_k_cf() { return poseidon_k_dense<T>() + (T - 1) * (T - 1); }
template <int T> constexpr int poseidon_k_tail() { return poseidon_k_cf<T>() + (T - 1); }
template <int T> constexpr int poseidon_k_m() { return poseidon_k_tail<T>() + 3 * T; }
template <int T> constexpr int poseidon_const_frs() { return poseidon_k_m<T>() + T * T; }

HZ_HD constexpr int poseidon_nsbox_rt(int t) {
    return 8 * t + (t == 2 ? 56 : t == 3 ? 57 : t == 4 ? 56 : t == 5 ? 60 : t == 6 ? 60 : 63);
}

struct NoSink {
    static constexpr bool kCanon = false;
    HZ_HD void operator()(int, const Fr&, const Fr&, const Fr&) const {}
};

template <class Sink>
HZ_HD Fr poseidon_sbox(const Fr& x, int k, Sink& sink) {
    if constexpr (Sink::kCanon) {
        const Fr x2 = fr_sqr(x);
        const Fr in2 = fr_canon_limbs(x2);
        const Fr in4 = fr_cond_sub_p_rare(fr_mul(x2, in2));
        const Fr out = fr_cond_sub_p_rare(fr_mul(in4, x));
        sink(k, in2, in4, out);
        return out;
    } else {
        const Fr x2 = fr_sqr(x);
        const Fr x4 = fr_sqr(x2);
        const Fr x5 = fr_mul(x4, x);
        sink(k, x2, x4, x5);
        return x5;
    }
}

template <int N>
HZ_HD Fr poseidon_row(const Fr* row, const Fr* st, const Fr* addend) {
    if constexpr (N <= 6) {
        return fr_dot<N>(row, st, addend);
    } else {
        return fr_add(fr_dot<4>(row, st, addend), fr_dot<N - 4>(row + 4, st + 4));
    }
}

template <int T>
HZ_HD void poseidon_rotate_in(Fr (&a)[T], const Fr& v) {
#pragma unroll
    for (int i = 0; i + 1 < T; i++) a[i] = a[i + 1];
    a[T - 1] = v;
}
template <int T, int NC>
HZ_HD void poseidon_mix_ark(Fr (&st)[T], const Fr* M, const Fr* Cn) {
    static_assert(NC == T || NC == 1, "constants for every lane or for lane 0 only");
    Fr o[T];
#pragma unroll
    for (int i = 0; i < T; i++) o[i] = st[i];
    if constexpr (NC == T) {
#pragma unroll 1
        for (int i = 0; i < T; i++) poseidon_rotate_in<T>(o, poseidon_row<T>(M + i * T, st, Cn + i));
    } else {
        poseidon_rotate_in<T>(o, poseidon_row<T>(M, st, Cn));
#pragma unroll 1
        for (int i = 1; i < T; i++) poseidon_rotate_in<T>(o, poseidon_row<T>(M + i * T, st, nullptr));
    }
#pragma unroll
    for (int i = 0; i < T; i++) st[i] = o[i];
}
template <int T, class Sink>
HZ_HD void poseidon_sbox_layer(Fr (&st)[T], int k, Sink& sink) {
#pragma unroll 1
    for (int j = 0; j < T; j++) poseidon_rotate_in<T>(st, poseidon_sbox(st[0], k + j, sink));
}

template <int T, class Sink>
HZ_HD Fr poseidon_hash(const Fr* in, const Fr* K, Sink& sink) {
    constexpr int RP = PoseidonCfg<T>::RP;
    const Fr* M = K + poseidon_k_m<T>();
    Fr st[T];
    st[0] = K[0];
#pragma unroll
    for (int j = 1; j < T; j++) st[j] = fr_add(in[j - 1], K[j]);
    int k = 0;
#pragma unroll 1
    for (int r = 0; r < 3; r++) {
        poseidon_sbox_layer<T>(st, k, sink);
        k += T;
        poseidon_mix_ark<T, T>(st, M, K + T * (r + 1));
    }
    poseidon_sbox_layer<T>(st, k, sink);
    k += T;
    poseidon_mix_ark<T, 1>(st, M, K + poseidon_k_e0<T>());
    const Fr* S = K + poseidon_k_part<T>();
    int lazy = 0;
#pragma unroll 1
    for (int r = 0; r + 1 < RP; r += 2) {
        Fr v[T + 1];
        v[0] = poseidon_sbox(st[0], k, sink);
#pragma unroll
        for (int j = 1; j < T; j++) v[j] = st[j];
        const Fr sa = poseidon_row<T>(S, v, S + T);
        v[T] = v[0];
        v[0] = poseidon_sbox(sa, k + 1, sink);
        k += 2;
        st[0] = poseidon_row<T + 1>(S + T + 1, v, S + 2 * T + 2);
        const Fr* CA = S + 2 * T + 3;
#pragma unroll
        for (int j = 1; j < T; j++) st[j] = fr_muladd2(CA[j - 1], v[T], CA[T - 1 + j - 1], v[0], st[j]);
        if (++lazy == 3) {
            lazy = 0;
#pragma unroll
            for (int j = 1; j < T; j++) st[j] = fr_cond_sub_4p(st[j]);
        }
        S += 4 * T + 1;
    }
    if constexpr (RP % 2 == 1) {
        st[0] = poseidon_sbox(st[0], k, sink);
        k += 1;
        const Fr s0 = poseidon_row<T>(S, st, S + 2 * T - 1);
#pragma unroll
        for (int j = 1; j < T; j++) st[j] = fr_muladd(S[T + j - 1], st[0], st[j]);
        st[0] = s0;
    }
    {
        Fr o[T - 1];
#pragma unroll
        for (int i = 0; i + 1 < T; i++) o[i] = st[i + 1];
#pragma unroll 1
        for (int i = 0; i + 1 < T; i++)
            poseidon_rotate_in<T - 1>(o, poseidon_row<T - 1>(K + poseidon_k_dense<T>() + i * (T - 1), st + 1, K + poseidon_k_cf<T>() + i));
#pragma unroll
        for (int i = 1; i < T; i++) st[i] = o[i - 1];
    }
#pragma unroll 1
    for (int r = 0; r < 3; r++) {
        poseidon_sbox_layer<T>(st, k, sink);
        k += T;
        poseidon_mix_ark<T, T>(st, M, K + poseidon_k_tail<T>() + T * r);
    }
    poseidon_sbox_layer<T>(st, k, sink);
    return poseidon_row<T>(M, st, nullptr);
}

}
```

Before: 1.640 million.

## Use linear-recurrence formulation for Poseidon T=3 partial rounds

For width 3, the partial rounds are rewritten as a linear recurrence over a sliding window of the last 2N+1 values: N entry rounds, then each round does one s-box and one (2N+1)-term dot product, then an exit matrix restores the state. New precomputed constant tables are appended for the T=3 parameter set, and poseidon_row gains a case for longer dot products. The aim is fewer field multiplications per partial round than the paired sparse-matrix scheme. In exchange the loop handles one round per iteration, uses a larger register window, and drops the lazy reduction tuning.

```diff
diff --git a/circuits_amd/csrc/gen/poseidon_consts.inc b/circuits_amd/csrc/gen/poseidon_consts.inc
--- a/circuits_amd/csrc/gen/poseidon_consts.inc
+++ b/circuits_amd/csrc/gen/poseidon_consts.inc
@@ -550,7 +550,7 @@
   {0x06f7520fu, 0x09d4f250u, 0x15681fe9u, 0x01fcd044u, 0x105154f2u, 0x1a33cff0u, 0x14edfb9fu, 0x19bb1130u, 0x0008a998u},
 };
 #define HZ_POSEIDON_RP_T2 56
-HZ_CONST_ARR uint32_t HZ_POSEIDON_K_T3[407][9] = {
+HZ_CONST_ARR uint32_t HZ_POSEIDON_K_T3[487][9] = {
   {0x06950af2u, 0x08df52acu, 0x1f463fb0u, 0x0afd92f8u, 0x14c68fb5u, 0x085357afu, 0x17f37f7du, 0x1a172af8u, 0x00219b98u},
   {0x14ac6331u, 0x19c5c962u, 0x14d4d232u, 0x1b75b979u, 0x05cb57afu, 0x1631c351u, 0x1539ab4eu, 0x0ae57f69u, 0x00221b93u},
   {0x0a11b110u, 0x0dfeef5cu, 0x0072b018u, 0x1dd64482u, 0x001637a2u, 0x1ccbb6f7u, 0x1bfe61e2u, 0x125c529fu, 0x0001ce06u},
@@ -958,8 +958,88 @@
   {0x0004eaddu, 0x05365bf4u, 0x0493016eu, 0x1d1a2414u, 0x0c60826du, 0x023b2076u, 0x026fd3e9u, 0x055a47d6u, 0x0021dc8bu},
   {0x17fddfa0u, 0x161a5176u, 0x030d78bau, 0x15ef8400u, 0x08d839abu, 0x1b2dce76u, 0x14b8a677u, 0x07c85cffu, 0x000877ecu},
   {0x0e5224f4u, 0x1e27ada2u, 0x1eb9ae97u, 0x0a2f7a59u, 0x1f07c890u, 0x1a2da267u, 0x05d3f5a1u, 0x11654cdeu, 0x000ba411u},
+  {0x0f9e7ad7u, 0x110388bbu, 0x0b23a8beu, 0x0d3738ecu, 0x067c9996u, 0x106d3f50u, 0x0b10e901u, 0x0ec1ca43u, 0x00185422u},
+  {0x1d808d1bu, 0x1da4b2b8u, 0x1a384bf5u, 0x0f4905bau, 0x03e20d93u, 0x0012de4fu, 0x121bce86u, 0x16d26544u, 0x000ade3au},
+  {0x132d35feu, 0x16391cd7u, 0x16fa00a5u, 0x0bb956dbu, 0x1caed5d5u, 0x1b6e4830u, 0x0a6f14e8u, 0x07466b6cu, 0x00191d6cu},
+  {0x012e70d0u, 0x0da73962u, 0x1ec66759u, 0x09107002u, 0x033f84eeu, 0x1399f16eu, 0x0226a56eu, 0x08d116b4u, 0x000e6296u},
+  {0x05212230u, 0x1c5e5216u, 0x117426b0u, 0x0de4f9e8u, 0x0851a05au, 0x18c6202bu, 0x09247701u, 0x110886d9u, 0x002cb167u},
+  {0x18349cb5u, 0x0e276a55u, 0x0cde03c9u, 0x0a96a06cu, 0x02315530u, 0x02cc974fu, 0x15fc8764u, 0x05814578u, 0x0014a31cu},
+  {0x0f9e7ad7u, 0x110388bbu, 0x0b23a8beu, 0x0d3738ecu, 0x067c9996u, 0x106d3f50u, 0x0b10e901u, 0x0ec1ca43u, 0x00185422u},
+  {0x0bb951acu, 0x06443faau, 0x17ed611cu, 0x1884421cu, 0x1afce51fu, 0x0efea9e7u, 0x147f1ed0u, 0x0c2df3cfu, 0x00136fbcu},
+  {0x1fe33105u, 0x0c4a3c3cu, 0x1c2cdf0fu, 0x041c6828u, 0x048b6c4au, 0x0719d197u, 0x123ecde6u, 0x05abf637u, 0x002ba99eu},
+  {0x13599399u, 0x141ae82bu, 0x13ee16cbu, 0x1358b994u, 0x1601460au, 0x144e8e2fu, 0x0bfd8788u, 0x17aa03a2u, 0x002ae961u},
+  {0x0d3bd08cu, 0x0feb7751u, 0x1d3846e5u, 0x1c5c2edbu, 0x0f46f214u, 0x0e48042cu, 0x02dcab7cu, 0x135dd023u, 0x002d03e8u},
+  {0x145ca2aeu, 0x0a83cb5bu, 0x1b380299u, 0x1b497ca9u, 0x0c5f7b57u, 0x0e04e7b0u, 0x0caa6f0au, 0x1609488bu, 0x001404e3u},
+  {0x0f9e7ad7u, 0x110388bbu, 0x0b23a8beu, 0x0d3738ecu, 0x067c9996u, 0x106d3f50u, 0x0b10e901u, 0x0ec1ca43u, 0x00185422u},
+  {0x0272b847u, 0x06346ef5u, 0x0c8ec1c1u, 0x035af7d1u, 0x15220e07u, 0x11e6f08du, 0x0f794481u, 0x0c04df9fu, 0x0003d716u},
+  {0x1345adcbu, 0x1fd8f332u, 0x1452973fu, 0x1cf4fd83u, 0x105c2158u, 0x0dd3cb9du, 0x09aa53d0u, 0x054d8d5au, 0x001658a7u},
+  {0x0b73dfaau, 0x0cfc3613u, 0x0c2d2fe1u, 0x17f31d9du, 0x02738eedu, 0x1556f082u, 0x0c6e8687u, 0x0300354eu, 0x001e5a4bu},
+  {0x05074a99u, 0x111317f4u, 0x014d238du, 0x064ca0e8u, 0x0d7bc44au, 0x0de87b5eu, 0x14f45ea5u, 0x1d6943d3u, 0x000b8751u},
+  {0x0c1f3472u, 0x131bb540u, 0x06139810u, 0x19c0e9f8u, 0x1f148210u, 0x160a67ffu, 0x044eda1bu, 0x0e2ad750u, 0x001a2252u},
+  {0x1a20a661u, 0x0981b885u, 0x06d79da7u, 0x08daa59au, 0x0380cec8u, 0x07ac5a3eu, 0x19c2fd4bu, 0x14196579u, 0x001456f9u},
+  {0x18a3393cu, 0x1c64921au, 0x086b2a4eu, 0x0395e07au, 0x03b08b3au, 0x15d09a8bu, 0x08f94d20u, 0x0b4ed1f4u, 0x002a1918u},
+  {0x07333fe1u, 0x1da032afu, 0x0b8dfefdu, 0x16cad880u, 0x0c7b630du, 0x136b6f07u, 0x07235290u, 0x0a519961u, 0x0004c677u},
+  {0x1209e59bu, 0x08e09132u, 0x18911f8du, 0x102fb855u, 0x19afe3f1u, 0x09e52054u, 0x053de6bcu, 0x10453383u, 0x00168c24u},
+  {0x16e75c61u, 0x1ccb11d5u, 0x033a9b20u, 0x057beb75u, 0x0dfad334u, 0x0d67d33cu, 0x085bc126u, 0x134f64e8u, 0x002df0ddu},
+  {0x1ad4cd74u, 0x09d30312u, 0x19b558f8u, 0x0431fc33u, 0x07b03d18u, 0x196db0cau, 0x144cbcb3u, 0x1c0bfe49u, 0x0023c4dfu},
+  {0x14a0ae83u, 0x0ff2d3d0u, 0x033ab1c2u, 0x1153c00du, 0x05bb0b4bu, 0x14a14cbbu, 0x1e2496a9u, 0x1cf85214u, 0x00216486u},
+  {0x1c44cbe3u, 0x1e6f6307u, 0x1736bc63u, 0x14569838u, 0x0fdfeb22u, 0x0a23bf4eu, 0x023c0d04u, 0x112bfeacu, 0x00109e18u},
+  {0x031a7275u, 0x1b956f2cu, 0x146e9fffu, 0x0d258020u, 0x176fc1f2u, 0x027b3e4cu, 0x14fb11aau, 0x0783c5ddu, 0x000d2811u},
+  {0x103335ffu, 0x0e239bb3u, 0x11949dc4u, 0x11c135eau, 0x096a1366u, 0x1968715eu, 0x1b956333u, 0x15e404d8u, 0x0012f076u},
+  {0x06030173u, 0x1a6a0215u, 0x16b6688du, 0x1b60bae1u, 0x129be973u, 0x1c324eb7u, 0x1b56844fu, 0x0502c84du, 0x000bca8fu},
+  {0x0ac00e1cu, 0x1852b7a5u, 0x1b4981deu, 0x1079c5f1u, 0x08ae0bf7u, 0x034a4e0au, 0x046af703u, 0x088a0d40u, 0x001a8ba1u},
+  {0x0268e2efu, 0x0dc0d572u, 0x014db6feu, 0x14fa667bu, 0x0725f8f0u, 0x1eae9144u, 0x1bcc388eu, 0x1a77fc9du, 0x00059f29u},
+  {0x1846ed9bu, 0x08e5a4b5u, 0x18e6d5cbu, 0x0bf2ebc8u, 0x17cdedc6u, 0x0057c320u, 0x0a7eb589u, 0x128f7f02u, 0x0002df9fu},
+  {0x17149ed8u, 0x199aac4fu, 0x00fe8d7bu, 0x15d246f7u, 0x131454fdu, 0x0ea94784u, 0x132ab7d9u, 0x080a2e05u, 0x00070d33u},
+  {0x1360c06du, 0x07c5a4cbu, 0x092d4859u, 0x1c636dffu, 0x0982a75bu, 0x071ad8e5u, 0x093f77d4u, 0x19fe3579u, 0x001080fcu},
+  {0x07a260ceu, 0x05fa6666u, 0x08783750u, 0x154f99b9u, 0x1de07510u, 0x154e6b50u, 0x09557be4u, 0x00df220bu, 0x001ebdaeu},
+  {0x06d9cbaeu, 0x026e7970u, 0x0e2f889eu, 0x10630129u, 0x16400b49u, 0x0856ac93u, 0x1f570e8du, 0x0108eb91u, 0x00274afbu},
+  {0x08b5363eu, 0x14c410a1u, 0x15b17f7eu, 0x006f94a4u, 0x1afbdf6eu, 0x0ebe7b11u, 0x0db265cbu, 0x18f9c23bu, 0x0007a3f2u},
+  {0x17e92553u, 0x15c8e7f8u, 0x1873dc56u, 0x097878c5u, 0x02fc9637u, 0x137d5e25u, 0x0675ed12u, 0x07d77dafu, 0x000c249fu},
+  {0x0f601b14u, 0x0bce4390u, 0x087462efu, 0x0f4cff79u, 0x1f3110f1u, 0x122c1eb4u, 0x1e01c90fu, 0x04de328au, 0x0028aea3u},
+  {0x1e8bb2ddu, 0x0c83d3cdu, 0x1bff9c4au, 0x02f2f366u, 0x019c7e88u, 0x11586a5bu, 0x018b3ad4u, 0x019bda88u, 0x001c72a8u},
+  {0x166d9447u, 0x01721438u, 0x0c7be5edu, 0x0b3ab98cu, 0x0553547bu, 0x1b93678au, 0x05965facu, 0x01332ae3u, 0x001b46b5u},
+  {0x1841d845u, 0x140a6b5eu, 0x06a55093u, 0x09a6d190u, 0x0d8779b1u, 0x00cee4efu, 0x0206aa73u, 0x1b616fadu, 0x001f0907u},
+  {0x034e3da2u, 0x151ad829u, 0x045d4be6u, 0x0b929088u, 0x018d122cu, 0x0b60dcc3u, 0x1c01e1f9u, 0x097a47ceu, 0x0012d9c4u},
+  {0x1d16119bu, 0x162aa171u, 0x1c9c0906u, 0x1128008fu, 0x1011c8e6u, 0x155feefeu, 0x00e6ec03u, 0x093e9863u, 0x000b7dd9u},
+  {0x04ab1ffdu, 0x0f0de809u, 0x0f746cf0u, 0x008abf95u, 0x1a73ce9bu, 0x021f8049u, 0x01f5ca30u, 0x09a64988u, 0x0009cf11u},
+  {0x15e7247au, 0x1f7e81ceu, 0x16ecbfc9u, 0x19b14a42u, 0x084e4275u, 0x1f4136a1u, 0x08d07e01u, 0x1220ae96u, 0x002965b7u},
+  {0x104bd884u, 0x1f4d07adu, 0x012adabdu, 0x1e8f8cdbu, 0x0411cbbcu, 0x1f8f5726u, 0x0f743a71u, 0x0d273966u, 0x001962c1u},
+  {0x1bc13fa3u, 0x00402db9u, 0x0a681102u, 0x0352b816u, 0x1dd6faafu, 0x000ea62fu, 0x0cac0c9bu, 0x01bc8604u, 0x0020b47cu},
+  {0x1fe24a3fu, 0x16860c73u, 0x1c0d24e0u, 0x0fbbb3d5u, 0x0436667au, 0x0ac480bfu, 0x0b3f1588u, 0x14f67abcu, 0x001efec3u},
+  {0x0478bba1u, 0x095c5b03u, 0x1c62cc8cu, 0x1c3c09a2u, 0x09636215u, 0x12d7f7fdu, 0x1dbc490du, 0x1f36e5d1u, 0x001c9e5du},
+  {0x19d43ca4u, 0x142a85c0u, 0x1a7baa83u, 0x1d528e53u, 0x04b7874du, 0x115ef445u, 0x0c2b384au, 0x1d6e7ac6u, 0x0015e411u},
+  {0x0bef0528u, 0x1e60ce0bu, 0x12625eb2u, 0x0f06c979u, 0x17bff821u, 0x1c4a80a2u, 0x132550c0u, 0x18ca2149u, 0x0012beacu},
+  {0x16ecf0a9u, 0x0ba29d55u, 0x19fc5003u, 0x016510afu, 0x1ee7cdb6u, 0x035f8d62u, 0x141e9b32u, 0x0f9d5485u, 0x00187ff6u},
+  {0x07452b1eu, 0x050b3ccau, 0x11869664u, 0x1f04ef75u, 0x0e3210d6u, 0x052baa1du, 0x0754b624u, 0x187e53c4u, 0x001cc402u},
+  {0x1ebe4524u, 0x1165f492u, 0x02aa3957u, 0x1e610304u, 0x1f733033u, 0x081ca6bbu, 0x111d1ecfu, 0x17b3a4fau, 0x001585b8u},
+  {0x1962c482u, 0x0110c899u, 0x009b3017u, 0x08f0a8d2u, 0x0b499af5u, 0x1270d168u, 0x18b7ec1eu, 0x106380e5u, 0x000f764du},
+  {0x010b5631u, 0x0a009882u, 0x1eeadd3fu, 0x01fd3930u, 0x0a9c2187u, 0x15f5d923u, 0x0abbbe81u, 0x1965b583u, 0x0028e7c2u},
+  {0x04028405u, 0x0d9d3a2fu, 0x0dd86c9cu, 0x0c73793cu, 0x1b491699u, 0x0ae48132u, 0x11b2507du, 0x0051efe5u, 0x001731c4u},
+  {0x0e5d3d55u, 0x1b4a68f8u, 0x0125da9cu, 0x0616ff3au, 0x17a894efu, 0x1255354eu, 0x140b0978u, 0x1b0bd271u, 0x002dba17u},
+  {0x184dd24fu, 0x087c83d1u, 0x060b14a1u, 0x060c28d4u, 0x14f6e1ffu, 0x1c5a591du, 0x1eed29beu, 0x0619afb5u, 0x001aa528u},
+  {0x07cd7674u, 0x1b0bd010u, 0x043db212u, 0x12244178u, 0x10a27a3au, 0x17a27951u, 0x1c41cb9du, 0x0fa88d30u, 0x002851f5u},
+  {0x04a857cdu, 0x0ed38054u, 0x0595c22du, 0x0854b125u, 0x0b7ebab9u, 0x0af5281du, 0x0ebed40cu, 0x1464a7ccu, 0x0006b887u},
+  {0x06a7141bu, 0x170f57fau, 0x15caa40du, 0x0cd5c528u, 0x1cd0ddccu, 0x1b694d4au, 0x1e688fd0u, 0x140949beu, 0x001ec366u},
+  {0x0e73a7a8u, 0x0c8e54a0u, 0x0a081b8eu, 0x177ac387u, 0x1ff2a46bu, 0x1071d805u, 0x07cfb61cu, 0x0e97f7d0u, 0x00078af2u},
+  {0x063c6323u, 0x07cc6228u, 0x1eb2ce8au, 0x09c405d0u, 0x130cc308u, 0x08f42781u, 0x036bc25au, 0x05070c93u, 0x000d6806u},
+  {0x19978954u, 0x07a59405u, 0x06011e3cu, 0x0db94457u, 0x021a540du, 0x08b0187fu, 0x0b7619dcu, 0x1b736fedu, 0x002d7d70u},
+  {0x17b7f285u, 0x0a72e51du, 0x1cfbd870u, 0x0cc34952u, 0x112168a3u, 0x0fe66800u, 0x0176bd8du, 0x00361bbau, 0x0021409au},
+  {0x11a798d9u, 0x00e0a46du, 0x0371bbf3u, 0x0ea5b3e4u, 0x110f30b0u, 0x016cc9e8u, 0x0227ea4bu, 0x1d4edd85u, 0x00140c14u},
+  {0x0a58d9aau, 0x0078ded9u, 0x030ae444u, 0x1ad7ebc0u, 0x1d419337u, 0x0966a2c5u, 0x15c72424u, 0x0a6b7f74u, 0x002ead58u},
+  {0x03f5e7f4u, 0x040d1f71u, 0x115aeefbu, 0x006f3cccu, 0x0d8e7bc4u, 0x0258d62bu, 0x160abb45u, 0x00cf4ab0u, 0x002d0f94u},
+  {0x17b7970au, 0x10735d21u, 0x1e784426u, 0x00c08ddau, 0x17ecd95eu, 0x0fe9e4c2u, 0x13036b64u, 0x0c7330d1u, 0x002719c0u},
+  {0x14b9baccu, 0x1add079eu, 0x1b2fa55du, 0x18f2b9e0u, 0x00b515c0u, 0x08be58aeu, 0x097fd2ffu, 0x120eeba2u, 0x000ba768u},
+  {0x022cde4au, 0x0049a8f3u, 0x1a54f0f4u, 0x199300b8u, 0x0ab0a299u, 0x0ad1534du, 0x137ce233u, 0x18d3b8a5u, 0x0010a225u},
+  {0x1971fb6eu, 0x0d8f34a5u, 0x1a50e001u, 0x04c86631u, 0x15c5922du, 0x09f7f723u, 0x03b40cb1u, 0x10f92fa6u, 0x00289362u},
+  {0x0a84e5aau, 0x1baff18fu, 0x021f1807u, 0x184e02e8u, 0x1634ee4eu, 0x10335d58u, 0x199f00a9u, 0x1ffd1e1bu, 0x001f3f7eu},
+  {0x02ffaf3au, 0x11d3984fu, 0x082869e6u, 0x1ed62941u, 0x138b7271u, 0x0fb41ebau, 0x1b972513u, 0x17fcbd3bu, 0x0013807au},
+  {0x16e2c9ddu, 0x108da0a7u, 0x06c0df95u, 0x081b05a4u, 0x0b62ee11u, 0x06b9c1c3u, 0x162aa04fu, 0x16d6c883u, 0x00054b85u},
+  {0x0b27abccu, 0x1e74a36au, 0x117635a9u, 0x1e787e6fu, 0x142f61cau, 0x0cf6f920u, 0x1e6abc93u, 0x0b27b379u, 0x00081f33u},
+  {0x1c5a33c1u, 0x0e487379u, 0x12f1d0d6u, 0x1e541e27u, 0x031bb29au, 0x093a6940u, 0x1f3c0355u, 0x0219ccccu, 0x000410c9u},
+  {0x0c586cabu, 0x177c59b4u, 0x030f7f82u, 0x0c7c8b35u, 0x029c9293u, 0x076616bcu, 0x01af66fau, 0x168b7e25u, 0x000a8584u},
 };
-HZ_CONST_ARR uint32_t HZ_POSEIDON_KW_T3[407][9] = {
+HZ_CONST_ARR uint32_t HZ_POSEIDON_KW_T3[487][9] = {
   {0x06950af2u, 0x08df52acu, 0x1f463fb0u, 0x0afd92f8u, 0x14c68fb5u, 0x085357afu, 0x17f37f7du, 0x1a172af8u, 0x00219b98u},
   {0x14ac6331u, 0x19c5c962u, 0x14d4d232u, 0x1b75b979u, 0x05cb57afu, 0x1631c351u, 0x1539ab4eu, 0x0ae57f69u, 0x00221b93u},
   {0x0a11b110u, 0x0dfeef5cu, 0x0072b018u, 0x1dd64482u, 0x001637a2u, 0x1ccbb6f7u, 0x1bfe61e2u, 0x125c529fu, 0x0001ce06u},
@@ -1367,6 +1447,86 @@
   {0x06ca4b2bu, 0x0f221bc1u, 0x192f0137u, 0x033b3288u, 0x113c2166u, 0x07e5114du, 0x08d44449u, 0x1771f3efu, 0x000e08d9u},
   {0x0686d883u, 0x004f59bdu, 0x1b05a390u, 0x0d931b7cu, 0x1494c930u, 0x17dcce38u, 0x17d324a5u, 0x09f221bfu, 0x002856b1u},
   {0x009c1bbau, 0x0bdaaccdu, 0x19620decu, 0x1ed4065bu, 0x1d8de23eu, 0x105fb12au, 0x00059d0fu, 0x14ff9303u, 0x0004a081u},
+  {0x1a4711d7u, 0x16699559u, 0x1c235d50u, 0x0b4e4a8eu, 0x14df94adu, 0x0965c795u, 0x1d7afd37u, 0x0342cc8du, 0x002d76dbu},
+  {0x1d808d1bu, 0x1da4b2b8u, 0x1a384bf5u, 0x0f4905bau, 0x03e20d93u, 0x0012de4fu, 0x121bce86u, 0x16d26544u, 0x000ade3au},
+  {0x132d35feu, 0x16391cd7u, 0x16fa00a5u, 0x0bb956dbu, 0x1caed5d5u, 0x1b6e4830u, 0x0a6f14e8u, 0x07466b6cu, 0x00191d6cu},
+  {0x012e70d0u, 0x0da73962u, 0x1ec66759u, 0x09107002u, 0x033f84eeu, 0x1399f16eu, 0x0226a56eu, 0x08d116b4u, 0x000e6296u},
+  {0x14725df5u, 0x1b005648u, 0x0162c706u, 0x0531cd6du, 0x02a601f6u, 0x165a1032u, 0x162de27fu, 0x05fe8aa5u, 0x002ddc1bu},
+  {0x1726ad0au, 0x1fd8b292u, 0x09a1fb0fu, 0x151b5e74u, 0x0fe81d33u, 0x06afb3b4u, 0x0d979567u, 0x02e791a9u, 0x000c050bu},
+  {0x1a4711d7u, 0x16699559u, 0x1c235d50u, 0x0b4e4a8eu, 0x14df94adu, 0x0965c795u, 0x1d7afd37u, 0x0342cc8du, 0x002d76dbu},
+  {0x0bb951acu, 0x06443faau, 0x17ed611cu, 0x1884421cu, 0x1afce51fu, 0x0efea9e7u, 0x147f1ed0u, 0x0c2df3cfu, 0x00136fbcu},
+  {0x1fe33105u, 0x0c4a3c3cu, 0x1c2cdf0fu, 0x041c6828u, 0x048b6c4au, 0x0719d197u, 0x123ecde6u, 0x05abf637u, 0x002ba99eu},
+  {0x13599399u, 0x141ae82bu, 0x13ee16cbu, 0x1358b994u, 0x1601460au, 0x144e8e2fu, 0x0bfd8788u, 0x17aa03a2u, 0x002ae961u},
+  {0x0413c3d3u, 0x00677053u, 0x0db32591u, 0x176f5823u, 0x00799ebdu, 0x16a26366u, 0x0fed863fu, 0x0e234eb9u, 0x000482feu},
+  {0x00500816u, 0x11dd74ccu, 0x102676c6u, 0x12dfe538u, 0x01fb533bu, 0x12b3051fu, 0x1410dc8fu, 0x19fad55bu, 0x002166d6u},
+  {0x1a4711d7u, 0x16699559u, 0x1c235d50u, 0x0b4e4a8eu, 0x14df94adu, 0x0965c795u, 0x1d7afd37u, 0x0342cc8du, 0x002d76dbu},
+  {0x0272b847u, 0x06346ef5u, 0x0c8ec1c1u, 0x035af7d1u, 0x15220e07u, 0x11e6f08du, 0x0f794481u, 0x0c04df9fu, 0x0003d716u},
+  {0x1345adcbu, 0x1fd8f332u, 0x1452973fu, 0x1cf4fd83u, 0x105c2158u, 0x0dd3cb9du, 0x09aa53d0u, 0x054d8d5au, 0x001658a7u},
+  {0x0b73dfaau, 0x0cfc3613u, 0x0c2d2fe1u, 0x17f31d9du, 0x02738eedu, 0x1556f082u, 0x0c6e8687u, 0x0300354eu, 0x001e5a4bu},
+  {0x05074a99u, 0x111317f4u, 0x014d238du, 0x064ca0e8u, 0x0d7bc44au, 0x0de87b5eu, 0x14f45ea5u, 0x1d6943d3u, 0x000b8751u},
+  {0x0c1f3472u, 0x131bb540u, 0x06139810u, 0x19c0e9f8u, 0x1f148210u, 0x160a67ffu, 0x044eda1bu, 0x0e2ad750u, 0x001a2252u},
+  {0x1a20a661u, 0x0981b885u, 0x06d79da7u, 0x08daa59au, 0x0380cec8u, 0x07ac5a3eu, 0x19c2fd4bu, 0x14196579u, 0x001456f9u},
+  {0x18a3393cu, 0x1c64921au, 0x086b2a4eu, 0x0395e07au, 0x03b08b3au, 0x15d09a8bu, 0x08f94d20u, 0x0b4ed1f4u, 0x002a1918u},
+  {0x07333fe1u, 0x1da032afu, 0x0b8dfefdu, 0x16cad880u, 0x0c7b630du, 0x136b6f07u, 0x07235290u, 0x0a519961u, 0x0004c677u},
+  {0x1209e59bu, 0x08e09132u, 0x18911f8du, 0x102fb855u, 0x19afe3f1u, 0x09e52054u, 0x053de6bcu, 0x10453383u, 0x00168c24u},
+  {0x16e75c61u, 0x1ccb11d5u, 0x033a9b20u, 0x057beb75u, 0x0dfad334u, 0x0d67d33cu, 0x085bc126u, 0x134f64e8u, 0x002df0ddu},
+  {0x1ad4cd74u, 0x09d30312u, 0x19b558f8u, 0x0431fc33u, 0x07b03d18u, 0x196db0cau, 0x144cbcb3u, 0x1c0bfe49u, 0x0023c4dfu},
+  {0x14a0ae83u, 0x0ff2d3d0u, 0x033ab1c2u, 0x1153c00du, 0x05bb0b4bu, 0x14a14cbbu, 0x1e2496a9u, 0x1cf85214u, 0x00216486u},
+  {0x1c44cbe3u, 0x1e6f6307u, 0x1736bc63u, 0x14569838u, 0x0fdfeb22u, 0x0a23bf4eu, 0x023c0d04u, 0x112bfeacu, 0x00109e18u},
+  {0x031a7275u, 0x1b956f2cu, 0x146e9fffu, 0x0d258020u, 0x176fc1f2u, 0x027b3e4cu, 0x14fb11aau, 0x0783c5ddu, 0x000d2811u},
+  {0x103335ffu, 0x0e239bb3u, 0x11949dc4u, 0x11c135eau, 0x096a1366u, 0x1968715eu, 0x1b956333u, 0x15e404d8u, 0x0012f076u},
+  {0x06030173u, 0x1a6a0215u, 0x16b6688du, 0x1b60bae1u, 0x129be973u, 0x1c324eb7u, 0x1b56844fu, 0x0502c84du, 0x000bca8fu},
+  {0x0ac00e1cu, 0x1852b7a5u, 0x1b4981deu, 0x1079c5f1u, 0x08ae0bf7u, 0x034a4e0au, 0x046af703u, 0x088a0d40u, 0x001a8ba1u},
+  {0x0268e2efu, 0x0dc0d572u, 0x014db6feu, 0x14fa667bu, 0x0725f8f0u, 0x1eae9144u, 0x1bcc388eu, 0x1a77fc9du, 0x00059f29u},
+  {0x1846ed9bu, 0x08e5a4b5u, 0x18e6d5cbu, 0x0bf2ebc8u, 0x17cdedc6u, 0x0057c320u, 0x0a7eb589u, 0x128f7f02u, 0x0002df9fu},
+  {0x17149ed8u, 0x199aac4fu, 0x00fe8d7bu, 0x15d246f7u, 0x131454fdu, 0x0ea94784u, 0x132ab7d9u, 0x080a2e05u, 0x00070d33u},
+  {0x1360c06du, 0x07c5a4cbu, 0x092d4859u, 0x1c636dffu, 0x0982a75bu, 0x071ad8e5u, 0x093f77d4u, 0x19fe3579u, 0x001080fcu},
+  {0x07a260ceu, 0x05fa6666u, 0x08783750u, 0x154f99b9u, 0x1de07510u, 0x154e6b50u, 0x09557be4u, 0x00df220bu, 0x001ebdaeu},
+  {0x06d9cbaeu, 0x026e7970u, 0x0e2f889eu, 0x10630129u, 0x16400b49u, 0x0856ac93u, 0x1f570e8du, 0x0108eb91u, 0x00274afbu},
+  {0x08b5363eu, 0x14c410a1u, 0x15b17f7eu, 0x006f94a4u, 0x1afbdf6eu, 0x0ebe7b11u, 0x0db265cbu, 0x18f9c23bu, 0x0007a3f2u},
+  {0x17e92553u, 0x15c8e7f8u, 0x1873dc56u, 0x097878c5u, 0x02fc9637u, 0x137d5e25u, 0x0675ed12u, 0x07d77dafu, 0x000c249fu},
+  {0x0f601b14u, 0x0bce4390u, 0x087462efu, 0x0f4cff79u, 0x1f3110f1u, 0x122c1eb4u, 0x1e01c90fu, 0x04de328au, 0x0028aea3u},
+  {0x1e8bb2ddu, 0x0c83d3cdu, 0x1bff9c4au, 0x02f2f366u, 0x019c7e88u, 0x11586a5bu, 0x018b3ad4u, 0x019bda88u, 0x001c72a8u},
+  {0x166d9447u, 0x01721438u, 0x0c7be5edu, 0x0b3ab98cu, 0x0553547bu, 0x1b93678au, 0x05965facu, 0x01332ae3u, 0x001b46b5u},
+  {0x1841d845u, 0x140a6b5eu, 0x06a55093u, 0x09a6d190u, 0x0d8779b1u, 0x00cee4efu, 0x0206aa73u, 0x1b616fadu, 0x001f0907u},
+  {0x034e3da2u, 0x151ad829u, 0x045d4be6u, 0x0b929088u, 0x018d122cu, 0x0b60dcc3u, 0x1c01e1f9u, 0x097a47ceu, 0x0012d9c4u},
+  {0x1d16119bu, 0x162aa171u, 0x1c9c0906u, 0x1128008fu, 0x1011c8e6u, 0x155feefeu, 0x00e6ec03u, 0x093e9863u, 0x000b7dd9u},
+  {0x04ab1ffdu, 0x0f0de809u, 0x0f746cf0u, 0x008abf95u, 0x1a73ce9bu, 0x021f8049u, 0x01f5ca30u, 0x09a64988u, 0x0009cf11u},
+  {0x15e7247au, 0x1f7e81ceu, 0x16ecbfc9u, 0x19b14a42u, 0x084e4275u, 0x1f4136a1u, 0x08d07e01u, 0x1220ae96u, 0x002965b7u},
+  {0x104bd884u, 0x1f4d07adu, 0x012adabdu, 0x1e8f8cdbu, 0x0411cbbcu, 0x1f8f5726u, 0x0f743a71u, 0x0d273966u, 0x001962c1u},
+  {0x1bc13fa3u, 0x00402db9u, 0x0a681102u, 0x0352b816u, 0x1dd6faafu, 0x000ea62fu, 0x0cac0c9bu, 0x01bc8604u, 0x0020b47cu},
+  {0x1fe24a3fu, 0x16860c73u, 0x1c0d24e0u, 0x0fbbb3d5u, 0x0436667au, 0x0ac480bfu, 0x0b3f1588u, 0x14f67abcu, 0x001efec3u},
+  {0x0478bba1u, 0x095c5b03u, 0x1c62cc8cu, 0x1c3c09a2u, 0x09636215u, 0x12d7f7fdu, 0x1dbc490du, 0x1f36e5d1u, 0x001c9e5du},
+  {0x19d43ca4u, 0x142a85c0u, 0x1a7baa83u, 0x1d528e53u, 0x04b7874du, 0x115ef445u, 0x0c2b384au, 0x1d6e7ac6u, 0x0015e411u},
+  {0x0bef0528u, 0x1e60ce0bu, 0x12625eb2u, 0x0f06c979u, 0x17bff821u, 0x1c4a80a2u, 0x132550c0u, 0x18ca2149u, 0x0012beacu},
+  {0x16ecf0a9u, 0x0ba29d55u, 0x19fc5003u, 0x016510afu, 0x1ee7cdb6u, 0x035f8d62u, 0x141e9b32u, 0x0f9d5485u, 0x00187ff6u},
+  {0x07452b1eu, 0x050b3ccau, 0x11869664u, 0x1f04ef75u, 0x0e3210d6u, 0x052baa1du, 0x0754b624u, 0x187e53c4u, 0x001cc402u},
+  {0x1ebe4524u, 0x1165f492u, 0x02aa3957u, 0x1e610304u, 0x1f733033u, 0x081ca6bbu, 0x111d1ecfu, 0x17b3a4fau, 0x001585b8u},
+  {0x1962c482u, 0x0110c899u, 0x009b3017u, 0x08f0a8d2u, 0x0b499af5u, 0x1270d168u, 0x18b7ec1eu, 0x106380e5u, 0x000f764du},
+  {0x010b5631u, 0x0a009882u, 0x1eeadd3fu, 0x01fd3930u, 0x0a9c2187u, 0x15f5d923u, 0x0abbbe81u, 0x1965b583u, 0x0028e7c2u},
+  {0x04028405u, 0x0d9d3a2fu, 0x0dd86c9cu, 0x0c73793cu, 0x1b491699u, 0x0ae48132u, 0x11b2507du, 0x0051efe5u, 0x001731c4u},
+  {0x0e5d3d55u, 0x1b4a68f8u, 0x0125da9cu, 0x0616ff3au, 0x17a894efu, 0x1255354eu, 0x140b0978u, 0x1b0bd271u, 0x002dba17u},
+  {0x184dd24fu, 0x087c83d1u, 0x060b14a1u, 0x060c28d4u, 0x14f6e1ffu, 0x1c5a591du, 0x1eed29beu, 0x0619afb5u, 0x001aa528u},
+  {0x07cd7674u, 0x1b0bd010u, 0x043db212u, 0x12244178u, 0x10a27a3au, 0x17a27951u, 0x1c41cb9du, 0x0fa88d30u, 0x002851f5u},
+  {0x04a857cdu, 0x0ed38054u, 0x0595c22du, 0x0854b125u, 0x0b7ebab9u, 0x0af5281du, 0x0ebed40cu, 0x1464a7ccu, 0x0006b887u},
+  {0x06a7141bu, 0x170f57fau, 0x15caa40du, 0x0cd5c528u, 0x1cd0ddccu, 0x1b694d4au, 0x1e688fd0u, 0x140949beu, 0x001ec366u},
+  {0x0e73a7a8u, 0x0c8e54a0u, 0x0a081b8eu, 0x177ac387u, 0x1ff2a46bu, 0x1071d805u, 0x07cfb61cu, 0x0e97f7d0u, 0x00078af2u},
+  {0x063c6323u, 0x07cc6228u, 0x1eb2ce8au, 0x09c405d0u, 0x130cc308u, 0x08f42781u, 0x036bc25au, 0x05070c93u, 0x000d6806u},
+  {0x19978954u, 0x07a59405u, 0x06011e3cu, 0x0db94457u, 0x021a540du, 0x08b0187fu, 0x0b7619dcu, 0x1b736fedu, 0x002d7d70u},
+  {0x17b7f285u, 0x0a72e51du, 0x1cfbd870u, 0x0cc34952u, 0x112168a3u, 0x0fe66800u, 0x0176bd8du, 0x00361bbau, 0x0021409au},
+  {0x11a798d9u, 0x00e0a46du, 0x0371bbf3u, 0x0ea5b3e4u, 0x110f30b0u, 0x016cc9e8u, 0x0227ea4bu, 0x1d4edd85u, 0x00140c14u},
+  {0x0a58d9aau, 0x0078ded9u, 0x030ae444u, 0x1ad7ebc0u, 0x1d419337u, 0x0966a2c5u, 0x15c72424u, 0x0a6b7f74u, 0x002ead58u},
+  {0x03f5e7f4u, 0x040d1f71u, 0x115aeefbu, 0x006f3cccu, 0x0d8e7bc4u, 0x0258d62bu, 0x160abb45u, 0x00cf4ab0u, 0x002d0f94u},
+  {0x0bd149bbu, 0x110115dbu, 0x06ac4f48u, 0x13303004u, 0x03e01978u, 0x04d13876u, 0x097c1bb8u, 0x1f6d6398u, 0x00300a70u},
+  {0x0750e964u, 0x01e30e2au, 0x0ec98b32u, 0x13ea39b1u, 0x1952ec54u, 0x108d7e37u, 0x0900da88u, 0x0d55fb72u, 0x0026de6cu},
+  {0x022cde4au, 0x0049a8f3u, 0x1a54f0f4u, 0x199300b8u, 0x0ab0a299u, 0x0ad1534du, 0x137ce233u, 0x18d3b8a5u, 0x0010a225u},
+  {0x1971fb6eu, 0x0d8f34a5u, 0x1a50e001u, 0x04c86631u, 0x15c5922du, 0x09f7f723u, 0x03b40cb1u, 0x10f92fa6u, 0x00289362u},
+  {0x125b52d8u, 0x17a26393u, 0x1d080d39u, 0x1439f182u, 0x02e21d11u, 0x1d5bd65eu, 0x079e0144u, 0x1cf8e8c4u, 0x0019c0b3u},
+  {0x1c194ce3u, 0x1085d973u, 0x0a42d924u, 0x13a63824u, 0x0d20119eu, 0x03402ec0u, 0x1d634d14u, 0x19767f1au, 0x00233951u},
+  {0x16e2c9ddu, 0x108da0a7u, 0x06c0df95u, 0x081b05a4u, 0x0b62ee11u, 0x06b9c1c3u, 0x162aa04fu, 0x16d6c883u, 0x00054b85u},
+  {0x0b27abccu, 0x1e74a36au, 0x117635a9u, 0x1e787e6fu, 0x142f61cau, 0x0cf6f920u, 0x1e6abc93u, 0x0b27b379u, 0x00081f33u},
+  {0x1c5a33c1u, 0x0e487379u, 0x12f1d0d6u, 0x1e541e27u, 0x031bb29au, 0x093a6940u, 0x1f3c0355u, 0x0219ccccu, 0x000410c9u},
+  {0x0c586cabu, 0x177c59b4u, 0x030f7f82u, 0x0c7c8b35u, 0x029c9293u, 0x076616bcu, 0x01af66fau, 0x168b7e25u, 0x000a8584u},
 };
 #define HZ_POSEIDON_RP_T3 57
 HZ_CONST_ARR uint32_t HZ_POSEIDON_K_T4[533][9] = {
diff --git a/circuits_amd/csrc/poseidon.h b/circuits_amd/csrc/poseidon.h
--- a/circuits_amd/csrc/poseidon.h
+++ b/circuits_amd/csrc/poseidon.h
@@ -5,12 +5,12 @@
 
 template <int T>
 struct PoseidonCfg;
-template <> struct PoseidonCfg<2> { static constexpr int RP = 56; };
-template <> struct PoseidonCfg<3> { static constexpr int RP = 57; };
-template <> struct PoseidonCfg<4> { static constexpr int RP = 56; };
-template <> struct PoseidonCfg<5> { static constexpr int RP = 60; };
-template <> struct PoseidonCfg<6> { static constexpr int RP = 60; };
-template <> struct PoseidonCfg<7> { static constexpr int RP = 63; };
+template <> struct PoseidonCfg<2> { static constexpr int RP = 56; static constexpr bool REC = false; };
+template <> struct PoseidonCfg<3> { static constexpr int RP = 57; static constexpr bool REC = true; };
+template <> struct PoseidonCfg<4> { static constexpr int RP = 56; static constexpr bool REC = false; };
+template <> struct PoseidonCfg<5> { static constexpr int RP = 60; static constexpr bool REC = false; };
+template <> struct PoseidonCfg<6> { static constexpr int RP = 60; static constexpr bool REC = false; };
+template <> struct PoseidonCfg<7> { static constexpr int RP = 63; static constexpr bool REC = false; };
 
 template <int T> constexpr int poseidon_rounds() { return 8 + PoseidonCfg<T>::RP; }
 template <int T> constexpr int poseidon_nsbox() { return 8 * T + PoseidonCfg<T>::RP; }
@@ -23,7 +23,12 @@
 template <int T> constexpr int poseidon_k_cf() { return poseidon_k_dense<T>() + (T - 1) * (T - 1); }
 template <int T> constexpr int poseidon_k_tail() { return poseidon_k_cf<T>() + (T - 1); }
 template <int T> constexpr int poseidon_k_m() { return poseidon_k_tail<T>() + 3 * T; }
-template <int T> constexpr int poseidon_const_frs() { return poseidon_k_m<T>() + T * T; }
+template <int T> constexpr int poseidon_k_entry() { return poseidon_k_m<T>() + T * T; }
+template <int T> constexpr int poseidon_k_rec() { return poseidon_k_entry<T>() + (T - 1) * 2 * T - (T - 1); }
+template <int T> constexpr int poseidon_k_e() { return poseidon_k_rec<T>() + 2 * T - 1; }
+template <int T> constexpr int poseidon_k_exit() { return poseidon_k_e<T>() + PoseidonCfg<T>::RP - (T - 1); }
+template <int T> constexpr int poseidon_k_cx() { return poseidon_k_exit<T>() + 2 * (T - 1) * (T - 1); }
+template <int T> constexpr int poseidon_const_frs() { return PoseidonCfg<T>::REC ? poseidon_k_cx<T>() + T - 1 : poseidon_k_entry<T>(); }
 
 HZ_HD constexpr int poseidon_nsbox_rt(int t) {
     return 8 * t + (t == 2 ? 56 : t == 3 ? 57 : t == 4 ? 56 : t == 5 ? 60 : t == 6 ? 60 : 63);
@@ -56,8 +61,10 @@
 HZ_HD Fr poseidon_row(const Fr* row, const Fr* st, const Fr* addend) {
     if constexpr (N <= 6) {
         return fr_dot<N>(row, st, addend);
-    } else {
+    } else if constexpr (N <= 8) {
         return fr_add(fr_dot<4>(row, st, addend), fr_dot<N - 4>(row + 4, st + 4));
+    } else {
+        return fr_add(fr_dot<6>(row, st, addend), poseidon_row<N - 6>(row + 6, st + 6, nullptr));
     }
 }
 
@@ -66,6 +73,13 @@
 #pragma unroll
     for (int i = 0; i + 1 < T; i++) a[i] = a[i + 1];
     a[T - 1] = v;
+}
+template <int FROM, int LEN, int N>
+HZ_HD void poseidon_window_in(Fr (&a)[N], const Fr& v) {
+    static_assert(FROM + LEN <= N, "queue inside the array");
+#pragma unroll
+    for (int i = FROM; i + 1 < FROM + LEN; i++) a[i] = a[i + 1];
+    a[FROM + LEN - 1] = v;
 }
 template <int T, int NC>
 HZ_HD void poseidon_mix_ark(Fr (&st)[T], const Fr* M, const Fr* Cn) {
@@ -88,6 +102,49 @@
 HZ_HD void poseidon_sbox_layer(Fr (&st)[T], int k, Sink& sink) {
 #pragma unroll 1
     for (int j = 0; j < T; j++) poseidon_rotate_in<T>(st, poseidon_sbox(st[0], k + j, sink));
+}
+
+template <int T, class Sink>
+HZ_HD void poseidon_partial_rec(Fr (&st)[T], const Fr* K, int& k, Sink& sink) {
+    constexpr int RP = PoseidonCfg<T>::RP;
+    constexpr int N = T - 1;
+    Fr w[2 * N + 1];
+#pragma unroll
+    for (int i = 0; i < 2 * N + 1; i++) w[i] = st[0];
+    const Fr* S = K + poseidon_k_entry<T>();
+#pragma unroll 1
+    for (int r = 0; r < N; r++) {
+        st[0] = poseidon_sbox(st[0], k, sink);
+        k += 1;
+        poseidon_window_in<0, N + 1>(w, st[0]);
+        const Fr x = poseidon_row<T>(S, st, S + T);
+        poseidon_window_in<N + 1, N>(w, x);
+        if (r + 1 < N) {
+#pragma unroll
+            for (int j = 1; j < T; j++) st[j] = fr_muladd(S[T + j], st[0], st[j]);
+        }
+        st[0] = x;
+        S += 2 * T;
+    }
+    const Fr* E = K + poseidon_k_e<T>();
+#pragma unroll 1
+    for (int r = N; r < RP; r++) {
+        poseidon_window_in<0, N + 1>(w, poseidon_sbox(w[2 * N], k, sink));
+        k += 1;
+        poseidon_window_in<N + 1, N>(w, poseidon_row<2 * N + 1>(K + poseidon_k_rec<T>(), w, E));
+        E += 1;
+    }
+    {
+        st[0] = w[2 * N];
+        Fr o[N];
+#pragma unroll
+        for (int i = 0; i < N; i++) o[i] = st[i + 1];
+#pragma unroll 1
+        for (int i = 0; i < N; i++)
+            poseidon_rotate_in<N>(o, poseidon_row<2 * N>(K + poseidon_k_exit<T>() + i * 2 * N, w + 1, K + poseidon_k_cx<T>() + i));
+#pragma unroll
+        for (int i = 1; i < T; i++) st[i] = o[i - 1];
+    }
 }
 
 template <int T, class Sink>
@@ -108,46 +165,50 @@
     poseidon_sbox_layer<T>(st, k, sink);
     k += T;
     poseidon_mix_ark<T, 1>(st, M, K + poseidon_k_e0<T>());
-    const Fr* S = K + poseidon_k_part<T>();
-    int lazy = 0;
-#pragma unroll 1
-    for (int r = 0; r + 1 < RP; r += 2) {
-        Fr v[T + 1];
-        v[0] = poseidon_sbox(st[0], k, sink);
-#pragma unroll
-        for (int j = 1; j < T; j++) v[j] = st[j];
-        const Fr sa = poseidon_row<T>(S, v, S + T);
-        v[T] = v[0];
-        v[0] = poseidon_sbox(sa, k + 1, sink);
-        k += 2;
-        st[0] = poseidon_row<T + 1>(S + T + 1, v, S + 2 * T + 2);
-        const Fr* CA = S + 2 * T + 3;
-#pragma unroll
-        for (int j = 1; j < T; j++) st[j] = fr_muladd2(CA[j - 1], v[T], CA[T - 1 + j - 1], v[0], st[j]);
-        if (++lazy == 3) {
-            lazy = 0;
-#pragma unroll
-            for (int j = 1; j < T; j++) st[j] = fr_cond_sub_4p(st[j]);
-        }
-        S += 4 * T + 1;
-    }
-    if constexpr (RP % 2 == 1) {
-        st[0] = poseidon_sbox(st[0], k, sink);
-        k += 1;
-        const Fr s0 = poseidon_row<T>(S, st, S + 2 * T - 1);
-#pragma unroll
-        for (int j = 1; j < T; j++) st[j] = fr_muladd(S[T + j - 1], st[0], st[j]);
-        st[0] = s0;
-    }
-    {
-        Fr o[T - 1];
-#pragma unroll
-        for (int i = 0; i + 1 < T; i++) o[i] = st[i + 1];
-#pragma unroll 1
-        for (int i = 0; i + 1 < T; i++)
-            poseidon_rotate_in<T - 1>(o, poseidon_row<T - 1>(K + poseidon_k_dense<T>() + i * (T - 1), st + 1, K + poseidon_k_cf<T>() + i));
-#pragma unroll
-        for (int i = 1; i < T; i++) st[i] = o[i - 1];
+    if constexpr (PoseidonCfg<T>::REC) {
+        poseidon_partial_rec<T>(st, K, k, sink);
+    } else {
+        const Fr* S = K + poseidon_k_part<T>();
+        int lazy = 0;
+#pragma unroll 1
+        for (int r = 0; r + 1 < RP; r += 2) {
+            Fr v[T + 1];
+            v[0] = poseidon_sbox(st[0], k, sink);
+#pragma unroll
+            for (int j = 1; j < T; j++) v[j] = st[j];
+            const Fr sa = poseidon_row<T>(S, v, S + T);
+            v[T] = v[0];
+            v[0] = poseidon_sbox(sa, k + 1, sink);
+            k += 2;
+            st[0] = poseidon_row<T + 1>(S + T + 1, v, S + 2 * T + 2);
+            const Fr* CA = S + 2 * T + 3;
+#pragma unroll
+            for (int j = 1; j < T; j++) st[j] = fr_muladd2(CA[j - 1], v[T], CA[T - 1 + j - 1], v[0], st[j]);
+            if (++lazy == 3) {
+                lazy = 0;
+#pragma unroll
+                for (int j = 1; j < T; j++) st[j] = fr_cond_sub_4p(st[j]);
+            }
+            S += 4 * T + 1;
+        }
+        if constexpr (RP % 2 == 1) {
+            st[0] = poseidon_sbox(st[0], k, sink);
+            k += 1;
+            const Fr s0 = poseidon_row<T>(S, st, S + 2 * T - 1);
+#pragma unroll
+            for (int j = 1; j < T; j++) st[j] = fr_muladd(S[T + j - 1], st[0], st[j]);
+            st[0] = s0;
+        }
+        {
+            Fr o[T - 1];
+#pragma unroll
+            for (int i = 0; i + 1 < T; i++) o[i] = st[i + 1];
+#pragma unroll 1
+            for (int i = 0; i + 1 < T; i++)
+                poseidon_rotate_in<T - 1>(o, poseidon_row<T - 1>(K + poseidon_k_dense<T>() + i * (T - 1), st + 1, K + poseidon_k_cf<T>() + i));
+#pragma unroll
+            for (int i = 1; i < T; i++) st[i] = o[i - 1];
+        }
     }
 #pragma unroll 1
     for (int r = 0; r < 3; r++) {
```

Measured after the change: 1.675 million, median of 6. 2.1% higher.
